# hygenie1228/PoseRisk_RELEASE

Hardware: AMD Instinct MI355X
Metric: frames/sec (224x224 crops) through SPIN ResNet-50 + regressor + SMPL LBS + REBA/RULA (higher is better)
Workload: dtype f32; 1 GPU; configs[1]: batch=64 random 224x224 crops per GPU, ResNet-50+SMPL fp32; global_batch=64, batches_in_flight=3, hipgraph_replay=False, exchange=none, dist_world_size=1

## Files before the change

include/poserisk_hip.h:

```cpp
#ifndef POSERISK_HIP_H
#define POSERISK_HIP_H

#include <stddef.h>
#include <stdint.h>

#ifdef __cplusplus
extern "C" {
#endif

typedef enum pr_status {
  PR_OK = 0,
  PR_ERR_INVALID = -1,
  PR_ERR_HIP = -2,
  PR_ERR_NO_DEVICE = -3,
  PR_ERR_CAPACITY = -4
} pr_status;

const char* pr_last_error(void);
int pr_abi_version(void);
const char* pr_build_info(void);

int pr_declare_stream(void* stream, int declared);

int pr_stem_pool_f32_nhwc(int device, const float* x_dev, const float* w_host, const float* bias_host, float* y_dev, int B,
                          int repeats, float* ms_out, void* stream);

typedef struct pr_hmr pr_hmr_t;

size_t pr_hmr_weight_floats(void);

enum { PR_CONV_FORM_DEFAULT = -1, PR_CONV_FORM_DIRECT = 0, PR_CONV_FORM_WINOGRAD_2X2 = 2, PR_CONV_FORM_WINOGRAD_4X4 = 4,
       PR_CONV_FORM_WINOGRAD_4X4_B = 5, PR_CONV_FORM_BUILTIN_DEFAULT = 5 };
int pr_hmr_create(int device, const float* weights_host, size_t n_floats, int max_batch,
                  int precision, int conv_form, pr_hmr_t** out);
int pr_hmr_destroy(pr_hmr_t* h);

int pr_hmr_forward(pr_hmr_t* h, const float* x_dev, int B, float* rotmat_dev, float* betas_dev,
                   float* cam_dev, float* xf_dev, float* pose6d_dev, void* stream);

int pr_hmr_set_streams(pr_hmr_t* h, int n_streams);

int pr_hmr_set_concurrency(pr_hmr_t* h, int n_in_flight);

int pr_hmr_profile_enable(pr_hmr_t* h, int on);
int pr_hmr_profile_read(pr_hmr_t* h, float* ms_per_layer_host, int* launches_per_layer_host,
                        double* flops_per_layer_per_frame_host, double* mfma_flops_per_layer_per_frame_host,
                        int n_layers);
int pr_hmr_num_conv_layers(void);
int pr_hmr_plan_counts(pr_hmr_t* h, int B, int* conv_launches, int* winograd_layers);
int pr_hmr_encode_until(pr_hmr_t* h, const float* x_dev, int B, int block, void* act_dev, void* stream);
int pr_hmr_regress_until(pr_hmr_t* h, const float* xf_dev, int B, int step, float* out_dev, void* stream);
int pr_hmr_conv_form(pr_hmr_t* h);

int pr_conv_num_tile_cfgs(void);
int pr_conv2d_nhwc(int device, const void* x_dev, const float* w_host, const float* bias_host,
                   const void* res_dev, void* y_dev, int B, int H, int W, int Cin, int Cin_real,
                   int Cout, int KH, int KW, int stride, int pad, int relu, int tile_cfg,
                   int precision, int repeats, float* ms_out, void* stream);

int pr_conv1x1_dual_nhwc(int device, const void* x1_dev, const float* w1_host, const void* x2_dev,
                         const float* w2_host, const float* bias_host, void* y_dev, int B, int Ho, int Wo,
                         int Cin1, int H2, int W2, int Cin2, int stride2, int Cout, int relu, int tile_cfg,
                         int precision, void* stream);

int pr_conv3x3_conv1x1_nhwc(int device, const void* x_dev, const float* w2_host, const float* b2_host,
                            const float* w3_host, const float* b3_host, const void* res_dev, void* y_dev,
                            int B, int H, int W, int Cin, int N3, int relu3, int precision, void* stream);

int pr_bottleneck_nhwc(int device, const void* x_dev, const float* w1_host, const float* b1_host, const float* w2_host,
                       const float* b2_host, const float* w3_host, const float* b3_host, const float* wd_host,
                       const float* bd_host, void* y_dev, int B, int H, int W, int repeats, float* ms_out, void* stream);

int pr_bottleneck128_nhwc(int device, const void* x_dev, const float* w1_host, const float* b1_host, const float* w2_host,
                          const float* b2_host, const float* w3_host, const float* b3_host, void* y_dev, int B, int H, int W,
                          int repeats, float* ms_out, void* stream);

int pr_bottleneck256_nhwc(int device, const void* x_dev, const float* w1_host, const float* b1_host, const float* w2_host,
                          const float* b2_host, const float* w3_host, const float* b3_host, void* y_dev, int B, int H, int W,
                          int repeats, float* ms_out, void* stream);

int pr_stem_pool_nhwc(int device, const void* x_dev, const float* w_host, const float* bias_host, void* y_dev, int B, int H,
                      int repeats, float* ms_out, void* stream);

int pr_crop_frames(const uint8_t* frames_dev, int F, int H, int W, int bgr, const int32_t* frame_idx_dev,
                   const float* bboxes_dev, int N, float scale, float* crops_dev, int32_t* status_dev,
                   void* stream);

int pr_rot6d_to_rotmat(const float* pose6d_dev, int N, float* rotmat_dev, void* stream);

int pr_pose_to_euler(const float* rotmat_dev, int N, float* axis_angle_dev, double* euler_deg_dev,
                     int32_t* status_dev, void* stream);
int pr_axis_angle_to_euler(const float* axis_angle_dev, int N, double* euler_deg_dev, int32_t* status_dev,
                           void* stream);

typedef struct pr_smpl pr_smpl_t;

int pr_smpl_create(int device, const float* v_template_host, const float* shapedirs_host,
                   const float* posedirs_host, const float* J_regressor_host,
                   const float* weights_host, const int32_t* parents_host,
                   const float* model_betas_host, int V, int J, int NB, int max_batch,
                   pr_smpl_t** out);
int pr_smpl_destroy(pr_smpl_t* h);

int pr_smpl_forward(pr_smpl_t* h, const float* pose_dev, const float* betas_dev,
                    const float* trans_dev, int B, int center_idx, float* verts_dev,
                    float* joints_dev, void* stream);

int pr_smpl_joint_cam(pr_smpl_t* h, float* axis_angle_dev, int N, float* joint_cam_dev,
                      float* verts_dev, void* stream);

typedef struct pr_reba_info {
  int32_t legs_bilateral;
  int32_t sitting;
  int32_t load_force;
  int32_t arm_supported_l;
  int32_t arm_supported_r;
  int32_t coupling;
  int32_t activity;
} pr_reba_info;

typedef struct pr_rula_info {
  int32_t arm_supported_l, arm_supported_r;
  int32_t a_muscle_l, a_muscle_r;
  int32_t a_load_l, a_load_r;
  int32_t legs_bilateral;
  int32_t b_muscle, b_load;
} pr_rula_info;

int pr_reba(const double* euler_deg_dev, int N, const pr_reba_info* info, int32_t* out_dev,
            void* stream);
int pr_rula(const double* euler_deg_dev, int N, const pr_rula_info* info, int32_t* out_dev,
            void* stream);

typedef struct pr_frames_out {
  float* rotmat;
  float* betas;
  float* cam;
  float* axis_angle;
  double* euler_deg;
  float* joint_cam;
  float* verts;
  int32_t* reba;
  int32_t* rula;
  int32_t* status;
} pr_frames_out;

int pr_frames_forward(pr_hmr_t* hmr, pr_smpl_t* smpl, const float* x_dev, int B,
                      const pr_reba_info* reba_info, const pr_rula_info* rula_info,
                      const pr_frames_out* out, void* stream);

typedef struct pr_render_args {
  const float* verts;
  const int32_t* faces;
  const float* cam;
  const float* bboxes;
  const uint8_t* frames;
  const int32_t* frame_idx;
  const int32_t* face_part;
  const uint8_t* part_rgb;
  uint8_t* out;
  int32_t* face_id;
  int32_t* vert_fx;
  int32_t* status;
  int N, V, F, P;
  int n_frames, H, W, bgr;
  float scale, alpha;
} pr_render_args;

size_t pr_render_workspace_bytes(int N, int V, int F, int H, int W);
int pr_render_overlay(const pr_render_args* args, void* workspace, size_t workspace_bytes, void* stream);

#ifdef __cplusplus
}
#endif
#endif
```

poserisk_release_amd/_lib.py:

```python
import ctypes as C
import os

HERE = os.path.dirname(os.path.abspath(__file__))
LIB_PATH = os.environ.get("POSERISK_LIB_PATH") or os.path.join(HERE, "libposerisk_hip.so")

ABI_VERSION = 13


class PoseRiskHipError(RuntimeError):
    pass


class RebaInfo(C.Structure):
    _fields_ = [(n, C.c_int32) for n in ("legs_bilateral", "sitting", "load_force", "arm_supported_l",
                                          "arm_supported_r", "coupling", "activity")]


class RulaInfo(C.Structure):
    _fields_ = [(n, C.c_int32) for n in ("arm_supported_l", "arm_supported_r", "a_muscle_l", "a_muscle_r",
                                          "a_load_l", "a_load_r", "legs_bilateral", "b_muscle", "b_load")]


class RenderArgs(C.Structure):
    _fields_ = [(n, C.c_void_p) for n in ("verts", "faces", "cam", "bboxes", "frames", "frame_idx", "face_part", "part_rgb",
                                           "out", "face_id", "vert_fx", "status")] + \
               [(n, C.c_int) for n in ("N", "V", "F", "P", "n_frames", "H", "W", "bgr")] + \
               [("scale", C.c_float), ("alpha", C.c_float)]


class FramesOut(C.Structure):
    _fields_ = [(n, C.c_void_p) for n in ("rotmat", "betas", "cam", "axis_angle", "euler_deg", "joint_cam",
                                           "verts", "reba", "rula", "status")]


_P = C.c_void_p
_I = C.c_int
SIGNATURES = {
    "pr_last_error": (C.c_char_p, []),
    "pr_abi_version": (_I, []),
    "pr_build_info": (C.c_char_p, []),
    "pr_declare_stream": (_I, [_P, _I]),
    "pr_hmr_weight_floats": (C.c_size_t, []),
    "pr_hmr_create": (_I, [_I, _P, C.c_size_t, _I, _I, _I, C.POINTER(_P)]),
    "pr_hmr_destroy": (_I, [_P]),
    "pr_hmr_forward": (_I, [_P, _P, _I, _P, _P, _P, _P, _P, _P]),
    "pr_hmr_set_streams": (_I, [_P, _I]),
    "pr_hmr_set_concurrency": (_I, [_P, _I]),
    "pr_hmr_profile_enable": (_I, [_P, _I]),
    "pr_hmr_profile_read": (_I, [_P, _P, _P, _P, _P, _I]),
    "pr_hmr_num_conv_layers": (_I, []),
    "pr_hmr_conv_form": (_I, [_P]),
    "pr_hmr_plan_counts": (_I, [_P, _I, C.POINTER(_I), C.POINTER(_I)]),
    "pr_hmr_encode_until": (_I, [_P, _P, _I, _I, _P, _P]),
    "pr_hmr_regress_until": (_I, [_P, _P, _I, _I, _P, _P]),
    "pr_conv_num_tile_cfgs": (_I, []),
    "pr_conv2d_nhwc": (_I, [_I, _P, _P, _P, _P, _P] + [_I] * 14 + [_P, _P]),
    "pr_conv1x1_dual_nhwc": (_I, [_I, _P, _P, _P, _P, _P, _P] + [_I] * 12 + [_P]),
    "pr_conv3x3_conv1x1_nhwc": (_I, [_I, _P, _P, _P, _P, _P, _P, _P] + [_I] * 7 + [_P]),
    "pr_bottleneck_nhwc": (_I, [_I, _P, _P, _P, _P, _P, _P, _P, _P, _P, _P, _I, _I, _I, _I, _P, _P]),
    "pr_bottleneck128_nhwc": (_I, [_I, _P, _P, _P, _P, _P, _P, _P, _P, _I, _I, _I, _I, _P, _P]),
    "pr_bottleneck256_nhwc": (_I, [_I, _P, _P, _P, _P, _P, _P, _P, _P, _I, _I, _I, _I, _P, _P]),
    "pr_stem_pool_nhwc": (_I, [_I, _P, _P, _P, _P, _I, _I, _I, _P, _P]),
    "pr_stem_pool_f32_nhwc": (_I, [_I, _P, _P, _P, _P, _I, _I, _P, _P]),
    "pr_crop_frames": (_I, [_P, _I, _I, _I, _I, _P, _P, _I, C.c_float, _P, _P, _P]),
    "pr_rot6d_to_rotmat": (_I, [_P, _I, _P, _P]),
    "pr_pose_to_euler": (_I, [_P, _I, _P, _P, _P, _P]),
    "pr_axis_angle_to_euler": (_I, [_P, _I, _P, _P, _P]),
    "pr_smpl_create": (_I, [_I, _P, _P, _P, _P, _P, _P, _P, _I, _I, _I, _I, C.POINTER(_P)]),
    "pr_smpl_destroy": (_I, [_P]),
    "pr_smpl_forward": (_I, [_P, _P, _P, _P, _I, _I, _P, _P, _P]),
    "pr_smpl_joint_cam": (_I, [_P, _P, _I, _P, _P, _P]),
    "pr_reba": (_I, [_P, _I, C.POINTER(RebaInfo), _P, _P]),
    "pr_rula": (_I, [_P, _I, C.POINTER(RulaInfo), _P, _P]),
    "pr_frames_forward": (_I, [_P, _P, _P, _I, C.POINTER(RebaInfo), C.POINTER(RulaInfo),
                               C.POINTER(FramesOut), _P]),
    "pr_render_workspace_bytes": (C.c_size_t, [_I, _I, _I, _I, _I]),
    "pr_render_overlay": (_I, [C.POINTER(RenderArgs), _P, C.c_size_t, _P]),
}

_lib = None


def load():
    global _lib
    if _lib is not None:
        return _lib
    if not os.path.exists(LIB_PATH):
        raise PoseRiskHipError(
            f"{LIB_PATH} is missing: build it with `python -m poserisk_release_amd.build` "
            "(there is no CPU fallback for the hot path)")
    import torch
    try:
        lib = C.CDLL(LIB_PATH)
    except OSError as e:
        raise PoseRiskHipError(f"cannot load {LIB_PATH}: {e}") from e
    for name, (res, args) in SIGNATURES.items():
        fn = getattr(lib, name)
        fn.restype = res
        fn.argtypes = args
    if lib.pr_abi_version() != ABI_VERSION:
        raise PoseRiskHipError(f"ABI version mismatch: library {lib.pr_abi_version()}, binding {ABI_VERSION}")
    _lib = lib
    return lib


def declare_stream(device=None):
    import torch
    lib = load()
    if torch.cuda.is_available():
        lib.pr_declare_stream(torch.cuda.current_stream(device).cuda_stream, 1)
    return lib


def check(status, what=""):
    if status != 0:
        msg = load().pr_last_error().decode("utf-8", "replace")
        raise PoseRiskHipError(f"{what} failed (status {status}): {msg}")


def reba_info_struct(info):
    return RebaInfo(int(info["Legs_bilateral_weight_bearing/walking"]), int(info["Sitting"]),
                    int(info["Load/Force Score"]), int(info["Arm_supported_leaning_L"]),
                    int(info["Arm_supported_leaning_R"]), int(info["Coupling"]), int(info["Activity_Score"]))


def rula_info_struct(info):
    return RulaInfo(int(info["Arm_supported_leaning_L"]), int(info["Arm_supported_leaning_R"]),
                    int(info["A_Muscle_use_L"]), int(info["A_Muscle_use_R"]), int(info["A_Load/Force_L"]),
                    int(info["A_Load/Force_R"]), int(info["Legs_bilateral_weight_bearing"]),
                    int(info["B_Muscle_use"]), int(info["B_Load/Force"]))
```

poserisk_release_amd/csrc/capi.hip:

```cpp
#include <vector>

#include "conv_igemm.h"
#include "frame_kernels.h"

namespace pr {
namespace {
thread_local std::string g_last_error;
thread_local bool g_stream_declared = false;
thread_local hipStream_t g_declared_stream = nullptr;
}
void declared_stream(bool* declared, hipStream_t* s) {
  *declared = g_stream_declared;
  *s = g_declared_stream;
}
void set_error(const char* fmt, ...) {
  char buf[1024];
  va_list ap;
  va_start(ap, fmt);
  vsnprintf(buf, sizeof buf, fmt, ap);
  va_end(ap);
  g_last_error = buf;
}
}

#define PR_STR_(x) #x
#define PR_STR(x) PR_STR_(x)

extern "C" {

const char* pr_last_error(void) { return pr::g_last_error.c_str(); }
int pr_abi_version(void) { return 13; }

int pr_declare_stream(void* stream, int declared) {
  pr::g_stream_declared = declared != 0;
  pr::g_declared_stream = declared ? (hipStream_t)stream : nullptr;
  return PR_OK;
}

const char* pr_build_info(void) {
  return "gfx950"
#ifdef PR_TIMING_HOOKS
         " +PR_TIMING_HOOKS(results may be wrong)"
#endif
#ifdef PR_EXPERIMENT
         " +PR_EXPERIMENT=" PR_STR(PR_EXPERIMENT)
#endif
#if !defined(PR_TIMING_HOOKS) && !defined(PR_EXPERIMENT)
         " release"
#endif
      ;
}

int pr_rot6d_to_rotmat(const float* pose6d_dev, int N, float* rotmat_dev, void* stream) {
  PR_REQUIRE(pose6d_dev && rotmat_dev && N >= 0, "pr_rot6d_to_rotmat: bad argument");
  return pr::launch_rot6d(pose6d_dev, rotmat_dev, (long)N * 24, (hipStream_t)stream);
}

int pr_pose_to_euler(const float* rotmat_dev, int N, float* axis_angle_dev, double* euler_deg_dev,
                     int32_t* status_dev, void* stream) {
  PR_REQUIRE(rotmat_dev && axis_angle_dev && euler_deg_dev && N >= 0, "pr_pose_to_euler: bad argument");
  return pr::launch_pose_to_euler(rotmat_dev, N, axis_angle_dev, euler_deg_dev, status_dev,
                                  (hipStream_t)stream);
}

int pr_axis_angle_to_euler(const float* axis_angle_dev, int N, double* euler_deg_dev, int32_t* status_dev,
                           void* stream) {
  PR_REQUIRE(axis_angle_dev && euler_deg_dev && N >= 0, "pr_axis_angle_to_euler: bad argument");
  return pr::launch_pose_to_euler(nullptr, N, const_cast<float*>(axis_angle_dev), euler_deg_dev, status_dev,
                                  (hipStream_t)stream);
}

int pr_reba(const double* euler_deg_dev, int N, const pr_reba_info* info, int32_t* out_dev, void* stream) {
  PR_REQUIRE(euler_deg_dev && info && out_dev && N >= 0, "pr_reba: bad argument");
  return pr::launch_reba(euler_deg_dev, N, *info, out_dev, (hipStream_t)stream);
}

int pr_rula(const double* euler_deg_dev, int N, const pr_rula_info* info, int32_t* out_dev, void* stream) {
  PR_REQUIRE(euler_deg_dev && info && out_dev && N >= 0, "pr_rula: bad argument");
  return pr::launch_rula(euler_deg_dev, N, *info, out_dev, (hipStream_t)stream);
}

int pr_crop_frames(const uint8_t* frames_dev, int F, int H, int W, int bgr, const int32_t* frame_idx_dev,
                   const float* bboxes_dev, int N, float scale, float* crops_dev, int32_t* status_dev,
                   void* stream) {
  PR_REQUIRE(frames_dev && bboxes_dev && crops_dev, "pr_crop_frames: null argument");
  PR_REQUIRE(F > 0 && H > 0 && W > 0 && H < 32768 && W < 32768 && N >= 0 && scale > 0, "pr_crop_frames: bad geometry");
  PR_REQUIRE(frame_idx_dev || N <= F, "pr_crop_frames: %d boxes for %d frames without a frame index", N, F);
  return pr::launch_crop_frames(frames_dev, F, H, W, bgr, frame_idx_dev, bboxes_dev, N, scale, crops_dev,
                                status_dev, (hipStream_t)stream);
}

int pr_conv_num_tile_cfgs(void) { return pr::conv_num_tile_cfgs(); }

int pr_conv2d_nhwc(int device, const void* x_dev, const float* w_host, const float* bias_host,
                   const void* res_dev, void* y_dev, int B, int H, int W, int Cin, int Cin_real, int Cout,
                   int KH, int KW, int stride, int pad, int relu, int tile_cfg, int precision, int repeats,
                   float* ms_out, void* stream) {
  using namespace pr;
  PR_REQUIRE(x_dev && w_host && y_dev, "pr_conv2d_nhwc: null argument");
  PR_REQUIRE(precision == 0 || precision == 1, "pr_conv2d_nhwc: precision %d unknown", precision);
  PR_REQUIRE(precision == 0 || Cin % 8 == 0, "pr_conv2d_nhwc: bf16 needs Cin %% 8 == 0");
  PR_REQUIRE(Cin_real > 0 && Cin_real <= Cin && Cout % 64 == 0, "pr_conv2d_nhwc: bad channels");
  PR_REQUIRE(stride > 0 && pad >= 0 && KH > 0 && KW > 0, "pr_conv2d_nhwc: bad geometry");
  DeviceGuard g(device);
  hipStream_t s = (hipStream_t)stream;
  PR_TRY(refuse_if_capturing(s, "stand-alone test entry"));
  ConvProblem p;
  p.B = B; p.H = H; p.W = W; p.Cin = Cin; p.Cout = Cout; p.KH = KH; p.KW = KW; p.stride = stride; p.pad = pad;
  p.Ho = (H + 2 * pad - KH) / stride + 1;
  p.Wo = (W + 2 * pad - KW) / stride + 1;
  p.relu = relu;
  PR_REQUIRE(p.Ho > 0 && p.Wo > 0, "pr_conv2d_nhwc: empty output");
  p.precision = precision;
  p.tune = conv_tuning_from_env();
  struct Scratch {
    float *wd = nullptr, *bd = nullptr, *work = nullptr, *slab = nullptr;
    int* tickets = nullptr;
    hipEvent_t e0 = nullptr, e1 = nullptr;
    ~Scratch() {
      if (slab) (void)hipFree(slab);
      if (tickets) (void)hipFree(tickets);
      if (wd) (void)hipFree(wd);
      if (bd) (void)hipFree(bd);
      if (work) (void)hipFree(work);
      if (e0) (void)hipEventDestroy(e0);
      if (e1) (void)hipEventDestroy(e1);
    }
  } sc;
  float *&wd = sc.wd, *&bd = sc.bd, *&work = sc.work;
  const bool wino = tile_cfg == -2 || tile_cfg == -4 || tile_cfg == -5;
  const int wino_m = -tile_cfg;
  if (wino) {
    PR_REQUIRE(precision == 0 && KH == 3 && KW == 3 && stride == 1 && pad == 1 && !res_dev && Cin == Cin_real &&
                   Cin % 32 == 0,
               "pr_conv2d_nhwc: tile_cfg -2 / -4 / -5 (Winograd) is for fp32 3x3 / stride 1 / pad 1 without residual, Cin %% 32 == 0");
    const int wn = conv_winograd_tile(wino_m) + 2;
    std::vector<float> u((size_t)wn * wn * Cout * Cin);
    conv_winograd_pack_weights(w_host, nullptr, Cout, Cin, wino_m, u.data());
    PR_HIP(hipMalloc(&wd, u.size() * sizeof(float)));
    PR_HIP(hipMemcpy(wd, u.data(), u.size() * sizeof(float), hipMemcpyHostToDevice));
    PR_HIP(hipMalloc(&work, std::max<size_t>(conv_winograd_work_floats(p, wino_m), 4) * sizeof(float)));
  } else if (precision == 1) {
    std::vector<unsigned short> packed((size_t)Cout * conv_kpad_bf16(p.K()));
    conv_pack_weights_bf16(w_host, nullptr, Cout, Cin_real, Cin, KH, KW, packed.data());
    PR_HIP(hipMalloc(&wd, packed.size() * 2));
    PR_HIP(hipMemcpy(wd, packed.data(), packed.size() * 2, hipMemcpyHostToDevice));
  } else {
    std::vector<float> packed((size_t)Cout * p.Kpad());
    conv_pack_weights(w_host, nullptr, Cout, Cin_real, Cin, KH, KW, packed.data());
    PR_HIP(hipMalloc(&wd, packed.size() * sizeof(float)));
    PR_HIP(hipMemcpy(wd, packed.data(), packed.size() * sizeof(float), hipMemcpyHostToDevice));
  }
  if (bias_host) {
    PR_HIP(hipMalloc(&bd, Cout * sizeof(float)));
    PR_HIP(hipMemcpy(bd, bias_host, Cout * sizeof(float), hipMemcpyHostToDevice));
  }
  p.x = (const float*)x_dev; p.w = wd; p.bias = bd; p.res = (const float*)res_dev; p.y = (float*)y_dev;
  int cfg = tile_cfg >= 0 ? tile_cfg : conv_pick_tile_cfg(p);
  if (tile_cfg > 200 && tile_cfg <= 208) {
    PR_REQUIRE(precision == 0, "pr_conv2d_nhwc: split-K is fp32 only");
    cfg = 8;
    p.splitk = tile_cfg - 200;
    const size_t tiles = (size_t)ceil_div(p.M(), 64) * (Cout / 64);
    PR_HIP(hipMalloc(&sc.slab, tiles * p.splitk * 4096 * sizeof(float)));
    PR_HIP(hipMalloc(&sc.tickets, tiles * sizeof(int)));
    p.split_slab = sc.slab;
    p.split_tickets = sc.tickets;
  }
  auto go = [&]() -> int { return wino ? conv_winograd_launch(p, wd, work, wino_m, s) : conv_launch(p, cfg, s); };
  int st = go();
  if (st == PR_OK && repeats > 0 && ms_out) {
    hipEvent_t &e0 = sc.e0, &e1 = sc.e1;
    PR_HIP(hipEventCreate(&e0));
    PR_HIP(hipEventCreate(&e1));
    PR_HIP(hipEventRecord(e0, s));
    for (int i = 0; i < repeats && st == PR_OK; ++i) st = go();
    PR_HIP(hipEventRecord(e1, s));
    PR_HIP(hipEventSynchronize(e1));
    float ms = 0.f;
    PR_HIP(hipEventElapsedTime(&ms, e0, e1));
    *ms_out = ms / repeats;
  }
  hipError_t e = hipStreamSynchronize(s);
  if (st != PR_OK) return st;
  PR_HIP(e);
  return PR_OK;
}

int pr_conv1x1_dual_nhwc(int device, const void* x1_dev, const float* w1_host, const void* x2_dev, const float* w2_host,
                         const float* bias_host, void* y_dev, int B, int Ho, int Wo, int Cin1, int H2, int W2, int Cin2,
                         int stride2, int Cout, int relu, int tile_cfg, int precision, void* stream) {
  using namespace pr;
  PR_REQUIRE(x1_dev && w1_host && x2_dev && w2_host && y_dev, "pr_conv1x1_dual_nhwc: null argument");
  PR_REQUIRE(precision == 0 || precision == 1, "pr_conv1x1_dual_nhwc: precision %d unknown", precision);
  const int kq = precision == 1 ? 64 : kConvBK;
  PR_REQUIRE(Cin1 > 0 && Cin2 > 0 && Cin1 % kq == 0 && Cin2 % kq == 0 && Cout % 64 == 0 && stride2 > 0,
             "pr_conv1x1_dual_nhwc: channels must be multiples of %d (Cout of 64)", kq);
  DeviceGuard g(device);
  hipStream_t s = (hipStream_t)stream;
  PR_TRY(refuse_if_capturing(s, "stand-alone test entry"));
  ConvProblem p;
  p.B = B; p.H = p.Ho = Ho; p.W = p.Wo = Wo; p.Cin = Cin1; p.Cout = Cout; p.KH = p.KW = 1; p.stride = 1; p.pad = 0;
  p.relu = relu; p.precision = precision;
  p.tune = conv_tuning_from_env();
  p.H2 = H2; p.W2 = W2; p.Cin2 = Cin2; p.stride2 = stride2;
  struct Scratch {
    float *wd = nullptr, *bd = nullptr;
    ~Scratch() {
      if (wd) (void)hipFree(wd);
      if (bd) (void)hipFree(bd);
    }
  } sc;
  const size_t K = (size_t)Cin1 + Cin2;
  if (precision == 1) {
    std::vector<unsigned short> a((size_t)Cout * Cin1), b((size_t)Cout * Cin2), packed((size_t)Cout * K);
    conv_pack_weights_bf16(w1_host, nullptr, Cout, Cin1, Cin1, 1, 1, a.data());
    conv_pack_weights_bf16(w2_host, nullptr, Cout, Cin2, Cin2, 1, 1, b.data());
    for (int o = 0; o < Cout; ++o) {
      memcpy(&packed[o * K], &a[(size_t)o * Cin1], (size_t)Cin1 * 2);
      memcpy(&packed[o * K + Cin1], &b[(size_t)o * Cin2], (size_t)Cin2 * 2);
    }
    PR_HIP(hipMalloc(&sc.wd, packed.size() * 2));
    PR_HIP(hipMemcpy(sc.wd, packed.data(), packed.size() * 2, hipMemcpyHostToDevice));
  } else {
    std::vector<float> packed((size_t)Cout * K);
    for (int o = 0; o < Cout; ++o) {
      memcpy(&packed[o * K], w1_host + (size_t)o * Cin1, (size_t)Cin1 * 4);
      memcpy(&packed[o * K + Cin1], w2_host + (size_t)o * Cin2, (size_t)Cin2 * 4);
    }
    PR_HIP(hipMalloc(&sc.wd, packed.size() * 4));
    PR_HIP(hipMemcpy(sc.wd, packed.data(), packed.size() * 4, hipMemcpyHostToDevice));
  }
  if (bias_host) {
    PR_HIP(hipMalloc(&sc.bd, Cout * sizeof(float)));
    PR_HIP(hipMemcpy(sc.bd, bias_host, Cout * sizeof(float), hipMemcpyHostToDevice));
  }
  p.x = (const float*)x1_dev; p.x2 = (const float*)x2_dev; p.w = sc.wd; p.bias = sc.bd; p.res = nullptr; p.y = (float*)y_dev;
  const int cfg = tile_cfg >= 0 ? tile_cfg : conv_pick_tile_cfg(p);
  const int st = conv_launch(p, cfg, s);
  const hipError_t e = hipStreamSynchronize(s);
  if (st != PR_OK) return st;
  PR_HIP(e);
  return PR_OK;
}

int pr_conv3x3_conv1x1_nhwc(int device, const void* x_dev, const float* w2_host, const float* b2_host,
                            const float* w3_host, const float* b3_host, const void* res_dev, void* y_dev, int B, int H,
                            int W, int Cin, int N3, int relu3, int precision, void* stream) {
  using namespace pr;
  PR_REQUIRE(x_dev && w2_host && b2_host && w3_host && b3_host && y_dev, "pr_conv3x3_conv1x1_nhwc: null argument");
  PR_REQUIRE(precision == 0 || precision == 1, "pr_conv3x3_conv1x1_nhwc: precision %d unknown", precision);
  PR_REQUIRE(Cin >= (precision ? 64 : 32) && (Cin & (Cin - 1)) == 0 && N3 > 0 && N3 % 64 == 0,
             "pr_conv3x3_conv1x1_nhwc: Cin must be a power of two >= 32 (bf16: 64), N3 a multiple of 64");
  DeviceGuard g(device);
  hipStream_t s = (hipStream_t)stream;
  PR_TRY(refuse_if_capturing(s, "stand-alone test entry"));
  struct Scratch {
    float* p[4] = {nullptr, nullptr, nullptr, nullptr};
    ~Scratch() {
      for (float* q : p)
        if (q) (void)hipFree(q);
    }
  } sc;
  ConvProblem p;
  p.B = B; p.H = p.Ho = H; p.W = p.Wo = W; p.Cin = Cin; p.Cout = 64; p.KH = p.KW = 3; p.stride = 1; p.pad = 1; p.relu = 1;
  p.precision = precision;
  p.tune = conv_tuning_from_env();
  std::vector<float> w2p, w3p;
  if (precision == 1) {
    std::vector<unsigned short> a((size_t)64 * conv_kpad_bf16(p.K())), b((size_t)N3 * 64);
    conv_pack_weights_bf16(w2_host, nullptr, 64, Cin, Cin, 3, 3, a.data());
    conv_pack_weights_bf16(w3_host, nullptr, N3, 64, 64, 1, 1, b.data());
    w2p.resize((a.size() + 1) / 2);
    w3p.resize((b.size() + 1) / 2);
    memcpy(w2p.data(), a.data(), a.size() * 2);
    memcpy(w3p.data(), b.data(), b.size() * 2);
  } else {
    w2p.resize((size_t)64 * p.Kpad());
    conv_pack_weights(w2_host, nullptr, 64, Cin, Cin, 3, 3, w2p.data());
    w3p.assign(w3_host, w3_host + (size_t)N3 * 64);
  }
  const size_t sizes[4] = {w2p.size(), 64, w3p.size(), (size_t)N3};
  const float* src[4] = {w2p.data(), b2_host, w3p.data(), b3_host};
  for (int i = 0; i < 4; ++i) {
    PR_HIP(hipMalloc(&sc.p[i], sizes[i] * sizeof(float)));
    PR_HIP(hipMemcpy(sc.p[i], src[i], sizes[i] * sizeof(float), hipMemcpyHostToDevice));
  }
  p.x = (const float*)x_dev; p.w = sc.p[0]; p.bias = sc.p[1]; p.w3 = sc.p[2]; p.bias3 = sc.p[3];
  p.res3 = (const float*)res_dev; p.y3 = (float*)y_dev;
  p.N3 = N3; p.relu3 = relu3;
  const int st = conv_launch(p, 8, s);
  const hipError_t e = hipStreamSynchronize(s);
  if (st != PR_OK) return st;
  PR_HIP(e);
  return PR_OK;
}

int pr_bottleneck_nhwc(int device, const void* x_dev, const float* w1_host, const float* b1_host, const float* w2_host,
                       const float* b2_host, const float* w3_host, const float* b3_host, const float* wd_host,
                       const float* bd_host, void* y_dev, int B, int H, int W, int repeats, float* ms_out, void* stream) {
  using namespace pr;
  PR_REQUIRE(x_dev && w1_host && b1_host && w2_host && b2_host && w3_host && b3_host && y_dev, "pr_bottleneck_nhwc: null argument");
  PR_REQUIRE(!wd_host == !bd_host, "pr_bottleneck_nhwc: the downsample branch needs both its weight and its bias");
  PR_REQUIRE(B >= 0 && H > 0 && W > 0, "pr_bottleneck_nhwc: bad geometry");
  const bool first = wd_host != nullptr;
  const int cin = first ? 64 : 256, k3 = first ? 128 : 64;
  DeviceGuard g(device);
  hipStream_t s = (hipStream_t)stream;
  PR_TRY(refuse_if_capturing(s, "stand-alone test entry"));
  struct Scratch {
    void* p[6] = {};
    hipEvent_t e0 = nullptr, e1 = nullptr;
    ~Scratch() {
      for (void* q : p)
        if (q) (void)hipFree(q);
      if (e0) (void)hipEventDestroy(e0);
      if (e1) (void)hipEventDestroy(e1);
    }
  } sc;
  std::vector<unsigned short> a1((size_t)64 * cin), a2((size_t)64 * 576), a3((size_t)256 * 64), ad((size_t)256 * 64),
      a3d((size_t)256 * k3), p1(a1.size()), p2(a2.size()), p3(a3d.size());
  conv_pack_weights_bf16(w1_host, nullptr, 64, cin, cin, 1, 1, a1.data());
  conv_pack_weights_bf16(w2_host, nullptr, 64, 64, 64, 3, 3, a2.data());
  conv_pack_weights_bf16(w3_host, nullptr, 256, 64, 64, 1, 1, a3.data());
  if (first) conv_pack_weights_bf16(wd_host, nullptr, 256, 64, 64, 1, 1, ad.data());
  for (int o = 0; o < 256; ++o) {
    memcpy(&a3d[(size_t)o * k3], &a3[(size_t)o * 64], 128);
    if (first) memcpy(&a3d[(size_t)o * k3 + 64], &ad[(size_t)o * 64], 128);
  }
  std::vector<float> b3(b3_host, b3_host + 256);
  if (first)
    for (int o = 0; o < 256; ++o) b3[o] = (float)((double)b3_host[o] + (double)bd_host[o]);
  bottleneck_pack_rows_bf16(a1.data(), 64, cin, p1.data());
  bottleneck_pack_rows_bf16(a2.data(), 64, 576, p2.data());
  bottleneck_pack_rows_bf16(a3d.data(), 256, k3, p3.data());
  const void* src[6] = {p1.data(), p2.data(), p3.data(), b1_host, b2_host, b3.data()};
  const size_t bytes[6] = {p1.size() * 2, p2.size() * 2, p3.size() * 2, 64 * 4, 64 * 4, 256 * 4};
  for (int i = 0; i < 6; ++i) {
    PR_HIP(hipMalloc(&sc.p[i], bytes[i]));
    PR_HIP(hipMemcpy(sc.p[i], src[i], bytes[i], hipMemcpyHostToDevice));
  }
  BottleneckProblem p;
  p.x = x_dev; p.y = y_dev; p.w1 = sc.p[0]; p.w2 = sc.p[1]; p.w3 = sc.p[2];
  p.b1 = (const float*)sc.p[3]; p.b2 = (const float*)sc.p[4]; p.b3 = (const float*)sc.p[5];
  p.B = B; p.H = H; p.W = W; p.first = first;
  int st = bottleneck_bf16_launch(p, s);
  if (st == PR_OK && repeats > 0 && ms_out) {
    PR_HIP(hipEventCreate(&sc.e0));
    PR_HIP(hipEventCreate(&sc.e1));
    PR_HIP(hipEventRecord(sc.e0, s));
    for (int i = 0; i < repeats && st == PR_OK; ++i) st = bottleneck_bf16_launch(p, s);
    PR_HIP(hipEventRecord(sc.e1, s));
    PR_HIP(hipEventSynchronize(sc.e1));
    float ms = 0.f;
    PR_HIP(hipEventElapsedTime(&ms, sc.e0, sc.e1));
    *ms_out = ms / repeats;
  }
  const hipError_t e = hipStreamSynchronize(s);
  if (st != PR_OK) return st;
  PR_HIP(e);
  return PR_OK;
}

int pr_bottleneck128_nhwc(int device, const void* x_dev, const float* w1_host, const float* b1_host, const float* w2_host,
                          const float* b2_host, const float* w3_host, const float* b3_host, void* y_dev, int B, int H, int W,
                          int repeats, float* ms_out, void* stream) {
  using namespace pr;
  PR_REQUIRE(x_dev && w1_host && b1_host && w2_host && b2_host && w3_host && b3_host && y_dev, "pr_bottleneck128_nhwc: null argument");
  PR_REQUIRE(B >= 0 && H > 0 && W > 0, "pr_bottleneck128_nhwc: bad geometry");
  DeviceGuard g(device);
  hipStream_t s = (hipStream_t)stream;
  PR_TRY(refuse_if_capturing(s, "stand-alone test entry"));
  struct Scratch {
    void* p[6] = {};
    hipEvent_t e0 = nullptr, e1 = nullptr;
    ~Scratch() {
      for (void* q : p)
        if (q) (void)hipFree(q);
      if (e0) (void)hipEventDestroy(e0);
      if (e1) (void)hipEventDestroy(e1);
    }
  } sc;
  std::vector<unsigned short> a1((size_t)128 * 512), a2((size_t)128 * 1152), a3((size_t)512 * 128), p1(a1.size()), p2(a2.size()),
      p3(a3.size());
  conv_pack_weights_bf16(w1_host, nullptr, 128, 512, 512, 1, 1, a1.data());
  conv_pack_weights_bf16(w2_host, nullptr, 128, 128, 128, 3, 3, a2.data());
  conv_pack_weights_bf16(w3_host, nullptr, 512, 128, 128, 1, 1, a3.data());
  bottleneck_pack_rows_bf16(a1.data(), 128, 512, p1.data());
  bottleneck_pack_rows_bf16(a2.data(), 128, 1152, p2.data());
  bottleneck_pack_rows_bf16(a3.data(), 512, 128, p3.data());
  const void* src[6] = {p1.data(), p2.data(), p3.data(), b1_host, b2_host, b3_host};
  const size_t bytes[6] = {p1.size() * 2, p2.size() * 2, p3.size() * 2, 128 * 4, 128 * 4, 512 * 4};
  for (int i = 0; i < 6; ++i) {
    PR_HIP(hipMalloc(&sc.p[i], bytes[i]));
    PR_HIP(hipMemcpy(sc.p[i], src[i], bytes[i], hipMemcpyHostToDevice));
  }
  BottleneckProblem p;
  p.x = x_dev; p.y = y_dev; p.w1 = sc.p[0]; p.w2 = sc.p[1]; p.w3 = sc.p[2];
  p.b1 = (const float*)sc.p[3]; p.b2 = (const float*)sc.p[4]; p.b3 = (const float*)sc.p[5];
  p.B = B; p.H = H; p.W = W; p.planes = 128; p.first = false;
  int st = bottleneck_bf16_launch(p, s);
  if (st == PR_OK && repeats > 0 && ms_out) {
    PR_HIP(hipEventCreate(&sc.e0));
    PR_HIP(hipEventCreate(&sc.e1));
    PR_HIP(hipEventRecord(sc.e0, s));
    for (int i = 0; i < repeats && st == PR_OK; ++i) st = bottleneck_bf16_launch(p, s);
    PR_HIP(hipEventRecord(sc.e1, s));
    PR_HIP(hipEventSynchronize(sc.e1));
    float ms = 0.f;
    PR_HIP(hipEventElapsedTime(&ms, sc.e0, sc.e1));
    *ms_out = ms / repeats;
  }
  const hipError_t e = hipStreamSynchronize(s);
  if (st != PR_OK) return st;
  PR_HIP(e);
  return PR_OK;
}

int pr_bottleneck256_nhwc(int device, const void* x_dev, const float* w1_host, const float* b1_host, const float* w2_host,
                          const float* b2_host, const float* w3_host, const float* b3_host, void* y_dev, int B, int H, int W,
                          int repeats, float* ms_out, void* stream) {
  using namespace pr;
  PR_REQUIRE(x_dev && w1_host && b1_host && w2_host && b2_host && w3_host && b3_host && y_dev, "pr_bottleneck256_nhwc: null argument");
  PR_REQUIRE(B >= 0 && H > 0 && W > 0, "pr_bottleneck256_nhwc: bad geometry");
  DeviceGuard g(device);
  hipStream_t s = (hipStream_t)stream;
  PR_TRY(refuse_if_capturing(s, "stand-alone test entry"));
  struct Scratch {
    void* p[6] = {};
    hipEvent_t e0 = nullptr, e1 = nullptr;
    ~Scratch() {
      for (void* q : p)
        if (q) (void)hipFree(q);
      if (e0) (void)hipEventDestroy(e0);
      if (e1) (void)hipEventDestroy(e1);
    }
  } sc;
  std::vector<unsigned short> a1((size_t)256 * 1024), a2((size_t)256 * 2304), a3((size_t)1024 * 256), p1(a1.size()), p2(a2.size()),
      p3(a3.size()), rows(a2.size());
  conv_pack_weights_bf16(w1_host, nullptr, 256, 1024, 1024, 1, 1, a1.data());
  conv_pack_weights_bf16(w2_host, nullptr, 256, 256, 256, 3, 3, a2.data());
  conv_pack_weights_bf16(w3_host, nullptr, 1024, 256, 256, 1, 1, a3.data());
  bottleneck_pack_rows_bf16(a1.data(), 256, 1024, p1.data());
  bottleneck_pack_rows_bf16(a2.data(), 256, 2304, rows.data());
  bottleneck256_pack_w2_frags_bf16(rows.data(), p2.data());
  bottleneck_pack_rows_bf16(a3.data(), 1024, 256, rows.data());
  bottleneck256_pack_w3_frags_bf16(rows.data(), p3.data());
  const void* src[6] = {p1.data(), p2.data(), p3.data(), b1_host, b2_host, b3_host};
  const size_t bytes[6] = {p1.size() * 2, p2.size() * 2, p3.size() * 2, 256 * 4, 256 * 4, 1024 * 4};
  for (int i = 0; i < 6; ++i) {
    PR_HIP(hipMalloc(&sc.p[i], bytes[i]));
    PR_HIP(hipMemcpy(sc.p[i], src[i], bytes[i], hipMemcpyHostToDevice));
  }
  BottleneckProblem p;
  p.x = x_dev; p.y = y_dev; p.w1 = sc.p[0]; p.w2 = sc.p[1]; p.w3 = sc.p[2];
  p.b1 = (const float*)sc.p[3]; p.b2 = (const float*)sc.p[4]; p.b3 = (const float*)sc.p[5];
  p.B = B; p.H = H; p.W = W; p.planes = 256; p.first = false;
  int st = bottleneck_bf16_launch(p, s);
  if (st == PR_OK && repeats > 0 && ms_out) {
    PR_HIP(hipEventCreate(&sc.e0));
    PR_HIP(hipEventCreate(&sc.e1));
    PR_HIP(hipEventRecord(sc.e0, s));
    for (int i = 0; i < repeats && st == PR_OK; ++i) st = bottleneck_bf16_launch(p, s);
    PR_HIP(hipEventRecord(sc.e1, s));
    PR_HIP(hipEventSynchronize(sc.e1));
    float ms = 0.f;
    PR_HIP(hipEventElapsedTime(&ms, sc.e0, sc.e1));
    *ms_out = ms / repeats;
  }
  const hipError_t e = hipStreamSynchronize(s);
  if (st != PR_OK) return st;
  PR_HIP(e);
  return PR_OK;
}

int pr_stem_pool_nhwc(int device, const void* x_dev, const float* w_host, const float* bias_host, void* y_dev, int B, int H,
                      int repeats, float* ms_out, void* stream) {
  using namespace pr;
  PR_REQUIRE(x_dev && w_host && bias_host && y_dev, "pr_stem_pool_nhwc: null argument");
  DeviceGuard g(device);
  hipStream_t s = (hipStream_t)stream;
  PR_TRY(refuse_if_capturing(s, "stand-alone test entry"));
  struct Scratch {
    void* p[2] = {};
    hipEvent_t e0 = nullptr, e1 = nullptr;
    ~Scratch() {
      for (void* q : p)
        if (q) (void)hipFree(q);
      if (e0) (void)hipEventDestroy(e0);
      if (e1) (void)hipEventDestroy(e1);
    }
  } sc;
  std::vector<unsigned short> packed((size_t)64 * 256);
  conv_pack_weights_bf16(w_host, nullptr, 64, 16, 16, 4, 4, packed.data());
  PR_HIP(hipMalloc(&sc.p[0], packed.size() * 2));
  PR_HIP(hipMemcpy(sc.p[0], packed.data(), packed.size() * 2, hipMemcpyHostToDevice));
  PR_HIP(hipMalloc(&sc.p[1], 64 * 4));
  PR_HIP(hipMemcpy(sc.p[1], bias_host, 64 * 4, hipMemcpyHostToDevice));
  int st = stem_pool_bf16_launch(x_dev, sc.p[0], (const float*)sc.p[1], y_dev, B, H, s);
  if (st == PR_OK && repeats > 0 && ms_out) {
    PR_HIP(hipEventCreate(&sc.e0));
    PR_HIP(hipEventCreate(&sc.e1));
    PR_HIP(hipEventRecord(sc.e0, s));
    for (int i = 0; i < repeats && st == PR_OK; ++i) st = stem_pool_bf16_launch(x_dev, sc.p[0], (const float*)sc.p[1], y_dev, B, H, s);
    PR_HIP(hipEventRecord(sc.e1, s));
    PR_HIP(hipEventSynchronize(sc.e1));
    float ms = 0.f;
    PR_HIP(hipEventElapsedTime(&ms, sc.e0, sc.e1));
    *ms_out = ms / repeats;
  }
  const hipError_t e = hipStreamSynchronize(s);
  if (st != PR_OK) return st;
  PR_HIP(e);
  return PR_OK;
}

int pr_stem_pool_f32_nhwc(int device, const float* x_dev, const float* w_host, const float* bias_host, float* y_dev, int B,
                          int repeats, float* ms_out, void* stream) {
  using namespace pr;
  PR_REQUIRE(x_dev && w_host && bias_host && y_dev, "pr_stem_pool_f32_nhwc: null argument");
  DeviceGuard g(device);
  hipStream_t s = (hipStream_t)stream;
  PR_TRY(refuse_if_capturing(s, "stand-alone test entry"));
  struct Scratch {
    void* p[2] = {};
    hipEvent_t e0 = nullptr, e1 = nullptr;
    ~Scratch() {
      for (void* q : p)
        if (q) (void)hipFree(q);
      if (e0) (void)hipEventDestroy(e0);
      if (e1) (void)hipEventDestroy(e1);
    }
  } sc;
  for (int o = 0; o < 64; ++o)
    for (int c12 = 0; c12 < 12; ++c12)
      for (int t = 0; t < 4; ++t) {
        const int sub = c12 / 3;
        const float top = w_host[((o * 12 + c12) * 4 + 0) * 4 + t], left = w_host[((o * 12 + c12) * 4 + t) * 4 + 0];
        PR_REQUIRE(((sub >> 1) != 0 || top == 0.f) && ((sub & 1) != 0 || left == 0.f),
                   "pr_stem_pool_f32_nhwc: the weights must be a 7x7 kernel in the 4x4 taps' 8x8 window (zero for tap row 0 / "
                   "sub-row 0 and for tap column 0 / sub-column 0); output channel %d, channel %d is not", o, c12);
      }
  std::vector<float> packed((size_t)64 * 192);
  conv_pack_weights(w_host, nullptr, 64, 12, 12, 4, 4, packed.data());
  PR_HIP(hipMalloc(&sc.p[0], packed.size() * 4));
  PR_HIP(hipMemcpy(sc.p[0], packed.data(), packed.size() * 4, hipMemcpyHostToDevice));
  PR_HIP(hipMalloc(&sc.p[1], 64 * 4));
  PR_HIP(hipMemcpy(sc.p[1], bias_host, 64 * 4, hipMemcpyHostToDevice));
  int st = stem_pool_f32_launch(x_dev, (const float*)sc.p[0], (const float*)sc.p[1], y_dev, B, s);
  if (st == PR_OK && repeats > 0 && ms_out) {
    PR_HIP(hipEventCreate(&sc.e0));
    PR_HIP(hipEventCreate(&sc.e1));
    PR_HIP(hipEventRecord(sc.e0, s));
    for (int i = 0; i < repeats && st == PR_OK; ++i) st = stem_pool_f32_launch(x_dev, (const float*)sc.p[0], (const float*)sc.p[1], y_dev, B, s);
    PR_HIP(hipEventRecord(sc.e1, s));
    PR_HIP(hipEventSynchronize(sc.e1));
    float ms = 0.f;
    PR_HIP(hipEventElapsedTime(&ms, sc.e0, sc.e1));
    *ms_out = ms / repeats;
  }
  const hipError_t e = hipStreamSynchronize(s);
  if (st != PR_OK) return st;
  PR_HIP(e);
  return PR_OK;
}

int pr_frames_forward(pr_hmr_t* hmr, pr_smpl_t* smpl, const float* x_dev, int B,
                      const pr_reba_info* reba_info, const pr_rula_info* rula_info,
                      const pr_frames_out* out, void* stream) {
  PR_REQUIRE(B >= 0, "pr_frames_forward: negative batch");
  if (B == 0) return PR_OK;
  PR_REQUIRE(hmr && smpl && x_dev && out, "pr_frames_forward: null argument");
  PR_REQUIRE(out->rotmat && out->axis_angle && out->euler_deg && out->joint_cam,
             "pr_frames_forward: rotmat, axis_angle, euler_deg and joint_cam are required");
  PR_REQUIRE((!out->reba || reba_info) && (!out->rula || rula_info), "pr_frames_forward: score output without info");
  PR_TRY(pr_hmr_forward(hmr, x_dev, B, out->rotmat, out->betas, out->cam, nullptr, nullptr, stream));
  PR_TRY(pr_pose_to_euler(out->rotmat, B, out->axis_angle, out->euler_deg, out->status, stream));
  PR_TRY(pr_smpl_joint_cam(smpl, out->axis_angle, B, out->joint_cam, out->verts, stream));
  if (out->reba) PR_TRY(pr_reba(out->euler_deg, B, reba_info, out->reba, stream));
  if (out->rula) PR_TRY(pr_rula(out->euler_deg, B, rula_info, out->rula, stream));
  return PR_OK;
}

}
```

poserisk_release_amd/csrc/conv_igemm.h:

```cpp
#pragma once
#include "common.h"
#include "host_plan.h"

namespace pr {


struct ConvTuning {
  int force_cfg = -1;
  int tail = 1;
  int tail_min_rounds = 2;
  int tail_max_rem = 128;
  int wino_vec = 2;
  int wino_bm = 64, wino_bn = 64;
  int wino_regw = 1;
  int regw_per_cu = 2;
  int regw_wt = 0, regw_wnb = 0;
  int regw_t = 0, regw_nb = 0;
  int bal_stages = 4;
};
ConvTuning conv_tuning_from_env();

struct ConvProblem {
  const float* x;
  const float* w;
  const float* bias;
  const float* res;
  float* y;
  int B, H, W, Cin, Ho, Wo, Cout, KH, KW, stride, pad;
  int relu;
  int precision = 0;
  int groups = 1;
  const float* x2 = nullptr;
  int H2 = 0, W2 = 0, Cin2 = 0, stride2 = 1;
  const float* w3 = nullptr;
  const float* bias3 = nullptr;
  const float* res3 = nullptr;
  float* y3 = nullptr;
  int N3 = 0, relu3 = 0;
  int splitk = 1;
  float* split_slab = nullptr;
  int* split_tickets = nullptr;
  ConvTuning tune;
  int M() const { return B * Ho * Wo; }
  int K() const { return KH * KW * Cin; }
  int Kpad() const { return ceil_div(K(), kConvBK) * kConvBK; }
  double flops() const { return 2.0 * (double)M() * (Cout * (K() + (x2 ? Cin2 : 0)) + (w3 ? (double)N3 * Cout : 0.0)); }
};

int conv_num_tile_cfgs();
const char* conv_tile_cfg_name(int cfg);
int conv_pick_tile_cfg(const ConvProblem& p);
int conv_launch(const ConvProblem& p, int cfg, hipStream_t stream);

int conv_fused3_launch(const ConvProblem& p, hipStream_t stream);

int conv_panel_launch(const ConvProblem& p, hipStream_t stream);

int conv_dma_launch(const ConvProblem& p, int BM, int BN, hipStream_t stream, int threads = 0);

int conv_dma_bf16_launch(const ConvProblem& p, int BM, int BN, hipStream_t stream, int threads = 0);
int conv_tile_dims(int cfg, int* BM, int* BN);

size_t conv_winograd_work_floats(const ConvProblem& p, int form);
int conv_winograd_launch(const ConvProblem& p, const float* u, float* work, int form, hipStream_t stream);

struct BottleneckProblem {
  const void* x = nullptr;
  void* y = nullptr;
  const void *w1 = nullptr, *w2 = nullptr, *w3 = nullptr;
  const float *b1 = nullptr, *b2 = nullptr, *b3 = nullptr;
  int B = 0, H = 0, W = 0, planes = 64;
  bool first = false;
  int lead_tiles = 2;
  double flops() const { return 2.0 * B * H * W * (double)planes * planes * (first ? 1 + 9 + 8 : 4 + 9 + 4); }
};
int bottleneck_bf16_launch(const BottleneckProblem& p, hipStream_t stream);
int bottleneck128_bf16_launch(const BottleneckProblem& p, hipStream_t stream);
int bottleneck256_bf16_launch(const BottleneckProblem& p, hipStream_t stream);

int stem_pool_bf16_launch(const void* x_s2d, const void* w, const float* bias, void* y, int B, int H, hipStream_t stream);

int stem_pool_f32_launch(const float* x_s2d, const float* w, const float* bias, float* y, int B, hipStream_t stream);

int expand_dual_bf16_launch(const void* t, const void* x2, const void* w, const float* bias, void* y, int B, int Ho, int Wo, int H2,
                            int W2, int stride2, int K1, int K2, int N, int relu, hipStream_t stream);
int expand_res_bf16_launch(const void* t, const void* w, const float* bias, const void* res, void* y, long M, int K, int N,
                           int relu, hipStream_t stream);

bool conv_bal_bf16_fits(const ConvProblem& p);
bool conv_bal_bf16_pays(const ConvProblem& p, int cus);
int conv_bal_bf16_launch(const ConvProblem& p, hipStream_t stream, int variant = 0);

bool conv_regw_f32_fits(const ConvProblem& p);
int conv_regw_f32_launch(const ConvProblem& p, hipStream_t stream);

}
```

poserisk_release_amd/csrc/conv_winograd.hip:

```cpp
#include <algorithm>

#include "conv_igemm.h"

namespace pr {
namespace {

using f32x4 = __attribute__((ext_vector_type(4))) float;

struct WinoArgs {
  const float* x;
  float* v;
  const float* m;
  const float* bias;
  float* y;
  int B, H, W, C, Cout, th, tw, relu;
  long P;
};

__global__ __launch_bounds__(256) void wino_input_transform(const WinoArgs a) {
  const int c4n = a.C >> 2;
  const long idx = xcd_contiguous_block(blockIdx.x, gridDim.x) * 256 + threadIdx.x;
  if (idx >= a.P * c4n) return;
  const long p = idx / c4n;
  const int c = (int)(idx - p * c4n) * 4;
  const int tx = (int)(p % a.tw);
  const long q = p / a.tw;
  const int ty = (int)(q % a.th), img = (int)(q / a.th);
  const int h0 = 2 * ty - 1, w0 = 2 * tx - 1;
  f32x4 d[4][4];
#pragma unroll
  for (int i = 0; i < 4; ++i)
#pragma unroll
    for (int j = 0; j < 4; ++j) {
      const int hi = h0 + i, wi = w0 + j;
      const bool ok = (unsigned)hi < (unsigned)a.H && (unsigned)wi < (unsigned)a.W;
      const f32x4 z = {0.f, 0.f, 0.f, 0.f};
      d[i][j] = ok ? *reinterpret_cast<const f32x4*>(a.x + (((long)img * a.H + hi) * a.W + wi) * a.C + c) : z;
    }
  f32x4 t[4][4];
#pragma unroll
  for (int j = 0; j < 4; ++j) {
    t[0][j] = d[0][j] - d[2][j];
    t[1][j] = d[1][j] + d[2][j];
    t[2][j] = d[2][j] - d[1][j];
    t[3][j] = d[1][j] - d[3][j];
  }
  const long gs = a.P * a.C;
  float* out = a.v + p * a.C + c;
#pragma unroll
  for (int i = 0; i < 4; ++i) {
    *reinterpret_cast<f32x4*>(out + (4 * i + 0) * gs) = t[i][0] - t[i][2];
    *reinterpret_cast<f32x4*>(out + (4 * i + 1) * gs) = t[i][1] + t[i][2];
    *reinterpret_cast<f32x4*>(out + (4 * i + 2) * gs) = t[i][2] - t[i][1];
    *reinterpret_cast<f32x4*>(out + (4 * i + 3) * gs) = t[i][1] - t[i][3];
  }
}

__global__ __launch_bounds__(256) void wino_output_transform(const WinoArgs a) {
  const int c4n = a.Cout >> 2;
  const long idx = xcd_contiguous_block(blockIdx.x, gridDim.x) * 256 + threadIdx.x;
  if (idx >= a.P * c4n) return;
  const long p = idx / c4n;
  const int c = (int)(idx - p * c4n) * 4;
  const int tx = (int)(p % a.tw);
  const long q = p / a.tw;
  const int ty = (int)(q % a.th), img = (int)(q / a.th);
  const long gs = a.P * a.Cout;
  const float* in = a.m + p * a.Cout + c;
  f32x4 m[4][4];
#pragma unroll
  for (int i = 0; i < 4; ++i)
#pragma unroll
    for (int j = 0; j < 4; ++j) m[i][j] = *reinterpret_cast<const f32x4*>(in + (4 * i + j) * gs);
  f32x4 s[2][4];
#pragma unroll
  for (int j = 0; j < 4; ++j) {
    s[0][j] = (m[0][j] + m[1][j]) + m[2][j];
    s[1][j] = (m[1][j] - m[2][j]) - m[3][j];
  }
  f32x4 b = {0.f, 0.f, 0.f, 0.f};
  if (a.bias) b = *reinterpret_cast<const f32x4*>(a.bias + c);
#pragma unroll
  for (int i = 0; i < 2; ++i) {
    const int ho = 2 * ty + i;
    if (ho >= a.H) continue;
    f32x4 o[2];
    o[0] = ((s[i][0] + s[i][1]) + s[i][2]) + b;
    o[1] = ((s[i][1] - s[i][2]) - s[i][3]) + b;
#pragma unroll
    for (int j = 0; j < 2; ++j) {
      const int wo = 2 * tx + j;
      if (wo >= a.W) continue;
      f32x4 v = o[j];
      if (a.relu) {
        v[0] = fmaxf(v[0], 0.f); v[1] = fmaxf(v[1], 0.f); v[2] = fmaxf(v[2], 0.f); v[3] = fmaxf(v[3], 0.f);
      }
      *reinterpret_cast<f32x4*>(a.y + (((long)img * a.H + ho) * a.W + wo) * a.Cout + c) = v;
    }
  }
}


using f32x2 = __attribute__((ext_vector_type(2))) float;

constexpr float kWa2 = kWa * kWa, kWb2 = kWb * kWb, kWab2 = kWa2 * kWb2, kWs2 = kWa2 + kWb2;

template <int PTS, typename V>
__device__ __forceinline__ void bt6(V& a0, V& a1, V& a2, V& a3, V& a4, V& a5) {
  const V d0 = a0, d1 = a1, d2 = a2, d3 = a3, d4 = a4, d5 = a5;
  if constexpr (PTS == 0) {
    a0 = 4.f * d0 - 5.f * d2 + d4;
    a1 = (d3 + d4) - 4.f * (d1 + d2);
    a2 = 4.f * (d1 - d2) + (d4 - d3);
    a3 = 2.f * (d3 - d1) + (d4 - d2);
    a4 = 2.f * (d1 - d3) + (d4 - d2);
    a5 = 4.f * d1 - 5.f * d3 + d5;
  } else {
    const V ea = d4 - kWb2 * d2, oa = kWa * (d3 - kWb2 * d1);
    const V eb = d4 - kWa2 * d2, ob = kWb * (d3 - kWa2 * d1);
    a0 = (kWab2 * d0 - kWs2 * d2) + d4;
    a1 = ea + oa;
    a2 = ea - oa;
    a3 = eb + ob;
    a4 = eb - ob;
    a5 = (kWab2 * d1 - kWs2 * d3) + d5;
  }
}

template <int PTS, typename V>
__global__ __launch_bounds__(256) void wino43_input_transform(const WinoArgs a) {
  constexpr int NC = sizeof(V) / 4;
  const int c2n = a.C / NC;
  const long idx = xcd_contiguous_block(blockIdx.x, gridDim.x) * 256 + threadIdx.x;
  if (idx >= a.P * c2n) return;
  const long p = idx / c2n;
  const int c = (int)(idx - p * c2n) * NC;
  const int tx = (int)(p % a.tw);
  const long q = p / a.tw;
  const int ty = (int)(q % a.th), img = (int)(q / a.th);
  const int h0 = 4 * ty - 1, w0 = 4 * tx - 1;
  V d[6][6];
#pragma unroll
  for (int i = 0; i < 6; ++i)
#pragma unroll
    for (int j = 0; j < 6; ++j) {
      const int hi = h0 + i, wi = w0 + j;
      const bool ok = (unsigned)hi < (unsigned)a.H && (unsigned)wi < (unsigned)a.W;
      V z;
#pragma unroll
      for (int e = 0; e < NC; ++e) z[e] = 0.f;
      d[i][j] = ok ? *reinterpret_cast<const V*>(a.x + (((long)img * a.H + hi) * a.W + wi) * a.C + c) : z;
    }
#pragma unroll
  for (int j = 0; j < 6; ++j) bt6<PTS>(d[0][j], d[1][j], d[2][j], d[3][j], d[4][j], d[5][j]);
#pragma unroll
  for (int i = 0; i < 6; ++i) bt6<PTS>(d[i][0], d[i][1], d[i][2], d[i][3], d[i][4], d[i][5]);
  const long gs = a.P * a.C;
  float* out = a.v + p * a.C + c;
#pragma unroll
  for (int i = 0; i < 6; ++i)
#pragma unroll
    for (int j = 0; j < 6; ++j) *reinterpret_cast<V*>(out + (6 * i + j) * gs) = d[i][j];
}

template <int PTS, typename V>
__device__ __forceinline__ void at6(const V m0, const V m1, const V m2, const V m3, const V m4, const V m5, V& o0, V& o1, V& o2, V& o3) {
  const V s12 = m1 + m2, d12 = m1 - m2, s34 = m3 + m4, d34 = m3 - m4;
  o0 = (m0 + s12) + s34;
  if constexpr (PTS == 0) {
    o1 = d12 + 2.f * d34;
    o2 = s12 + 4.f * s34;
    o3 = (d12 + 8.f * d34) + m5;
  } else {
    o1 = kWa * d12 + kWb * d34;
    o2 = kWa2 * s12 + kWb2 * s34;
    o3 = ((kWa2 * kWa) * d12 + (kWb2 * kWb) * d34) + m5;
  }
}

template <int PTS, typename V>
__global__ __launch_bounds__(256) void wino43_output_transform(const WinoArgs a) {
  constexpr int NC = sizeof(V) / 4;
  const int c2n = a.Cout / NC;
  const long idx = xcd_contiguous_block(blockIdx.x, gridDim.x) * 256 + threadIdx.x;
  if (idx >= a.P * c2n) return;
  const long p = idx / c2n;
  const int c = (int)(idx - p * c2n) * NC;
  const int tx = (int)(p % a.tw);
  const long q = p / a.tw;
  const int ty = (int)(q % a.th), img = (int)(q / a.th);
  const long gs = a.P * a.Cout;
  const float* in = a.m + p * a.Cout + c;
  V s[4][6];
#pragma unroll
  for (int j = 0; j < 6; ++j) {
    V m[6];
#pragma unroll
    for (int i = 0; i < 6; ++i) m[i] = *reinterpret_cast<const V*>(in + (6 * i + j) * gs);
    at6<PTS>(m[0], m[1], m[2], m[3], m[4], m[5], s[0][j], s[1][j], s[2][j], s[3][j]);
  }
  V b;
#pragma unroll
  for (int e = 0; e < NC; ++e) b[e] = 0.f;
  if (a.bias) b = *reinterpret_cast<const V*>(a.bias + c);
#pragma unroll
  for (int i = 0; i < 4; ++i) {
    const int ho = 4 * ty + i;
    V o[4];
    at6<PTS>(s[i][0], s[i][1], s[i][2], s[i][3], s[i][4], s[i][5], o[0], o[1], o[2], o[3]);
    if (ho >= a.H) continue;
#pragma unroll
    for (int j = 0; j < 4; ++j) {
      const int wo = 4 * tx + j;
      if (wo >= a.W) continue;
      V v = o[j] + b;
      if (a.relu) {
#pragma unroll
        for (int e = 0; e < NC; ++e) v[e] = fmaxf(v[e], 0.f);
      }
      *reinterpret_cast<V*>(a.y + (((long)img * a.H + ho) * a.W + wo) * a.Cout + c) = v;
    }
  }
}

long wino_tiles(const ConvProblem& p, int m) { return (long)p.B * ((p.H + m - 1) / m) * ((p.W + m - 1) / m); }

}

size_t conv_winograd_work_floats(const ConvProblem& p, int form) {
  const int m = conv_winograd_tile(form);
  return (size_t)(m + 2) * (m + 2) * wino_tiles(p, m) * ((size_t)p.Cin + p.Cout);
}

int conv_winograd_launch(const ConvProblem& p, const float* u, float* work, int form, hipStream_t stream) {
  PR_REQUIRE(form == 2 || form == 4 || form == 5, "winograd: form %d (2 = F(2x2), 4 = F(4x4), 5 = F(4x4) on the points 0, +-11/16, +-3/2)", form);
  const int m_out = conv_winograd_tile(form);
  PR_REQUIRE(p.precision == 0 && p.KH == 3 && p.KW == 3 && p.stride == 1 && p.pad == 1 && !p.res,
             "winograd: 3x3 / stride 1 / pad 1 fp32 convolutions without residual only");
  PR_REQUIRE(p.Cin % kConvBK == 0 && p.Cout % 64 == 0, "winograd: Cin %% 32 and Cout %% 64 (got %d, %d)", p.Cin, p.Cout);
  PR_REQUIRE(p.x && p.y && u && work, "winograd: null tensor");
  if (p.B == 0) return PR_OK;
  const int n2 = (m_out + 2) * (m_out + 2);
  WinoArgs a;
  a.x = p.x; a.bias = p.bias; a.y = p.y;
  a.B = p.B; a.H = p.H; a.W = p.W; a.C = p.Cin; a.Cout = p.Cout; a.relu = p.relu;
  a.th = (p.H + m_out - 1) / m_out; a.tw = (p.W + m_out - 1) / m_out;
  a.P = wino_tiles(p, m_out);
  a.v = work;
  float* m = work + (size_t)n2 * a.P * p.Cin;
  a.m = m;
  PR_REQUIRE(a.P * std::max(p.Cin, p.Cout) < (1L << 29), "winograd: %ld tiles are too many for one launch", a.P);
  const bool wide = m_out == 4 && p.tune.wino_vec == 4;
  const int per = m_out == 4 ? (wide ? 4 : 2) : 4;
  const long n_in = a.P * (p.Cin / per), n_out = a.P * (p.Cout / per);
  if (form == 5 && wide) hipLaunchKernelGGL((wino43_input_transform<1, f32x4>), dim3((unsigned)ceil_div(n_in, 256L)), dim3(256), 0, stream, a);
  else if (form == 5) hipLaunchKernelGGL((wino43_input_transform<1, f32x2>), dim3((unsigned)ceil_div(n_in, 256L)), dim3(256), 0, stream, a);
  else if (m_out == 4 && wide) hipLaunchKernelGGL((wino43_input_transform<0, f32x4>), dim3((unsigned)ceil_div(n_in, 256L)), dim3(256), 0, stream, a);
  else if (m_out == 4) hipLaunchKernelGGL((wino43_input_transform<0, f32x2>), dim3((unsigned)ceil_div(n_in, 256L)), dim3(256), 0, stream, a);
  else hipLaunchKernelGGL(wino_input_transform, dim3((unsigned)ceil_div(n_in, 256L)), dim3(256), 0, stream, a);
  PR_TRY(check_launch("wino_input_transform"));
  ConvProblem g;
  g.x = work; g.w = u; g.bias = nullptr; g.res = nullptr; g.y = m;
  g.B = (int)a.P; g.H = g.W = g.Ho = g.Wo = 1; g.Cin = p.Cin; g.Cout = p.Cout;
  g.KH = g.KW = 1; g.stride = 1; g.pad = 0; g.relu = 0; g.precision = 0;
  g.groups = n2;
  g.tune = p.tune;
  PR_REQUIRE(p.Cout % p.tune.wino_bn == 0, "winograd: Cout %d is not a multiple of the grouped GEMM's tile N %d", p.Cout, p.tune.wino_bn);
  if (p.tune.wino_regw && conv_regw_f32_fits(g)) PR_TRY(conv_regw_f32_launch(g, stream));
  else PR_TRY(conv_dma_launch(g, p.tune.wino_bm, p.tune.wino_bn, stream, 256));
  if (form == 5 && wide) hipLaunchKernelGGL((wino43_output_transform<1, f32x4>), dim3((unsigned)ceil_div(n_out, 256L)), dim3(256), 0, stream, a);
  else if (form == 5) hipLaunchKernelGGL((wino43_output_transform<1, f32x2>), dim3((unsigned)ceil_div(n_out, 256L)), dim3(256), 0, stream, a);
  else if (m_out == 4 && wide) hipLaunchKernelGGL((wino43_output_transform<0, f32x4>), dim3((unsigned)ceil_div(n_out, 256L)), dim3(256), 0, stream, a);
  else if (m_out == 4) hipLaunchKernelGGL((wino43_output_transform<0, f32x2>), dim3((unsigned)ceil_div(n_out, 256L)), dim3(256), 0, stream, a);
  else hipLaunchKernelGGL(wino_output_transform, dim3((unsigned)ceil_div(n_out, 256L)), dim3(256), 0, stream, a);
  return check_launch("wino_output_transform");
}

}
```

poserisk_release_amd/csrc/hmr.hip:

```cpp
#include <algorithm>
#include <cmath>
#include <cstdlib>
#include <cstring>
#include <memory>
#include <vector>

#include "conv_igemm.h"
#include "frame_kernels.h"

struct pr_hmr : pr::HmrPlan {
  int device = 0;
  pr::ConvTuning tune;
  float* split_slab[8] = {};
  int* split_tickets[8] = {};
  std::vector<float*> dev_allocs;
  static constexpr int kMaxChunks = pr::kHmrMaxChunks;
  int n_chunks = 1;
  int chunk_cap = 0;
  float* act[kMaxChunks][6] = {};
  float* wino_work[kMaxChunks] = {};
  hipStream_t streams[kMaxChunks] = {};
  hipEvent_t ev_fork = nullptr;
  hipEvent_t ev_join[kMaxChunks] = {};
  std::vector<float*> act_allocs;
  bool profile = false;
  std::vector<float> prof_ms;
  std::vector<int> prof_n;
  std::vector<std::pair<hipEvent_t, hipEvent_t>> pending;
  std::vector<int> pending_layer;
};

namespace pr {
namespace {

struct DeviceSink : PlanSink {
  pr_hmr* h;
  explicit DeviceSink(pr_hmr* handle) : h(handle) {}
  int upload(const void* host, size_t bytes, float** out) override {
    float* d = nullptr;
    PR_HIP(hipMalloc(&d, std::max<size_t>(bytes, 16)));
    h->dev_allocs.push_back(d);
    PR_HIP(hipMemcpy(d, host, bytes, hipMemcpyHostToDevice));
    *out = d;
    return PR_OK;
  }
  int zeros(size_t bytes, float** out) override {
    float* d = nullptr;
    PR_HIP(hipMalloc(&d, std::max<size_t>(bytes, 16)));
    h->dev_allocs.push_back(d);
    PR_HIP(hipMemset(d, 0, std::max<size_t>(bytes, 16)));
    *out = d;
    return PR_OK;
  }
};

int set_chunks(pr_hmr* h, int n) {
  PR_REQUIRE(n >= 1 && n <= pr_hmr::kMaxChunks, "hmr: stream count %d out of range 1..%d", n, pr_hmr::kMaxChunks);
  PR_HIP(hipDeviceSynchronize());
  for (float* p : h->act_allocs) (void)hipFree(p);
  h->act_allocs.clear();
  h->n_chunks = n;
  h->chunk_cap = hmr_chunk_cap(h->max_batch, n);
  const HmrChunkSizes z = hmr_chunk_sizes(*h, h->chunk_cap);
  for (int c = 0; c < n; ++c) {
    for (int i = 0; i <= 5; ++i) {
      float* d = nullptr;
      PR_HIP(hipMalloc(&d, (i == 0 ? z.act0_floats : z.act_floats) * sizeof(float)));
      h->act_allocs.push_back(d);
      h->act[c][i] = d;
    }
    if (z.wino_floats) {
      float* d = nullptr;
      PR_HIP(hipMalloc(&d, z.wino_floats * sizeof(float)));
      h->act_allocs.push_back(d);
      h->wino_work[c] = d;
    }
    if (z.slab_floats) {
      float* d = nullptr;
      PR_HIP(hipMalloc(&d, z.slab_floats * sizeof(float)));
      h->act_allocs.push_back(d);
      h->split_slab[c] = d;
      PR_HIP(hipMalloc(&d, z.tickets * sizeof(int)));
      h->act_allocs.push_back(d);
      h->split_tickets[c] = reinterpret_cast<int*>(d);
    }
    if (n > 1 && !h->streams[c]) PR_HIP(hipStreamCreateWithFlags(&h->streams[c], hipStreamNonBlocking));
    if (n > 1 && !h->ev_join[c]) PR_HIP(hipEventCreateWithFlags(&h->ev_join[c], hipEventDisableTiming));
  }
  if (n > 1 && !h->ev_fork) PR_HIP(hipEventCreateWithFlags(&h->ev_fork, hipEventDisableTiming));
  return PR_OK;
}

ConvProblem conv_problem(const pr_hmr* h, const ConvSpec& c, int chunk, int B) {
  ConvProblem p;
  p.x = h->act[chunk][c.in_buf];
  p.w = c.w;
  p.bias = c.bias;
  p.res = c.res_buf >= 0 ? h->act[chunk][c.res_buf] : nullptr;
  p.y = h->act[chunk][c.out_buf];
  p.B = B; p.H = c.H; p.W = c.W; p.Cin = c.Cin; p.Ho = c.Ho(); p.Wo = c.Wo(); p.Cout = c.Cout;
  p.KH = p.KW = c.k; p.stride = c.stride; p.pad = c.pad; p.relu = c.relu;
  p.precision = h->precision;
  p.tune = h->tune;
  if (c.in2_buf >= 0) {
    p.x2 = h->act[chunk][c.in2_buf];
    p.H2 = p.W2 = c.H2; p.Cin2 = c.Cin2; p.stride2 = c.stride2;
  }
  if (c.splitk > 1) {
    p.splitk = c.splitk;
    p.split_slab = h->split_slab[chunk];
    p.split_tickets = h->split_tickets[chunk];
  }
  if (c.w3 && c.out3_buf >= 0) {
    p.w3 = c.w3; p.bias3 = c.bias3; p.N3 = c.N3; p.relu3 = 1;
    p.res3 = c.res3_buf >= 0 ? h->act[chunk][c.res3_buf] : nullptr;
    p.y3 = h->act[chunk][c.out3_buf];
  }
  return p;
}

int fc_launch(const pr_hmr* h, const FcSpec& fc, const float* x, const float* res, float* y, int B, bool use_bias,
              hipStream_t s) {
  if (!h->fc_tiles) return launch_fc_rows16(x, fc.w, use_bias ? fc.bias : nullptr, res, y, B, fc.N, fc.K, s, h->fc_shape);
  ConvProblem p;
  p.x = x; p.w = fc.w; p.bias = use_bias ? fc.bias : nullptr; p.res = res; p.y = y;
  p.B = B; p.H = p.W = p.Ho = p.Wo = 1; p.Cin = fc.K; p.Cout = fc.N;
  p.KH = p.KW = 1; p.stride = 1; p.pad = 0; p.relu = 0;
  p.tune = h->tune;
  return conv_launch(p, conv_pick_tile_cfg(p), s);
}


struct ChunkRun {
  int chunk;
  const float* x;
  int b;
  float* xf_out;
  hipStream_t s;
  void* tap = nullptr;
};

size_t block_frame_elems(int k) {
  if (k == 0) return (size_t)56 * 56 * 64;
  const int L = k <= 3 ? 0 : k <= 7 ? 1 : k <= 13 ? 2 : 3, hw = 56 >> L;
  return (size_t)hw * hw * (256 << L);
}

int encode_chunks(pr_hmr* h, const ChunkRun* runs, int n, int stop_block = -1) {
  const bool bf = h->precision == 1;
  for (int i = 0; i < n; ++i) {
    if (h->stem_s2d) {
      if (bf) PR_TRY(launch_nchw3_to_s2d16_bf16(runs[i].x, h->act[runs[i].chunk][0], runs[i].b, kImg, kImg, runs[i].s));
      else PR_TRY(launch_nchw3_to_s2d12(runs[i].x, h->act[runs[i].chunk][0], runs[i].b, kImg, kImg, runs[i].s));
    } else {
      if (bf) PR_TRY(launch_nchw3_to_nhwc8_bf16(runs[i].x, h->act[runs[i].chunk][0], runs[i].b, kImg, kImg, runs[i].s));
      else PR_TRY(launch_nchw3_to_nhwc4(runs[i].x, h->act[runs[i].chunk][0], runs[i].b, kImg, kImg, runs[i].s));
    }
  }
  auto fused_pays = [&](int b) { return hmr_fused3_pays(b, h->cus); };
  size_t skip_until[pr_hmr::kMaxChunks] = {};
  for (size_t ci = 0; ci < h->convs.size(); ++ci) {
    ConvSpec& c = h->convs[ci];
    const int li = c.layer;
    const pr::HmrPlan::FusedBlock* alt = nullptr;
    for (const pr::HmrPlan::FusedBlock& fb : h->fused3)
      if (fb.first == ci) alt = &fb;
    for (int i = 0; i < n; ++i) {
      const ChunkRun& r = runs[i];
      if (ci < skip_until[i]) continue;
      if (alt && fused_pays(r.b)) {
        BottleneckProblem bp;
        bp.x = h->act[r.chunk][alt->blk.in_buf]; bp.y = h->act[r.chunk][alt->blk.out_buf];
        bp.w1 = alt->blk.w; bp.w2 = alt->blk.w2b; bp.w3 = alt->blk.w3;
        bp.b1 = alt->blk.bias; bp.b2 = alt->blk.bias2b; bp.b3 = alt->blk.bias3;
        bp.B = r.b; bp.H = alt->blk.H; bp.W = alt->blk.W; bp.planes = alt->blk.bneck_planes; bp.first = false;
        if (h->profile) {
          hipEvent_t e0, e1;
          PR_HIP(hipEventCreate(&e0));
          PR_HIP(hipEventCreate(&e1));
          PR_HIP(hipEventRecord(e0, r.s));
          PR_TRY(bottleneck_bf16_launch(bp, r.s));
          PR_HIP(hipEventRecord(e1, r.s));
          h->pending.emplace_back(e0, e1);
          h->pending_layer.push_back(alt->blk.layer);
        } else {
          PR_TRY(bottleneck_bf16_launch(bp, r.s));
        }
        skip_until[i] = ci + 3;
        continue;
      }
      ConvProblem p = c.bneck_planes ? ConvProblem{} : conv_problem(h, c, r.chunk, r.b);
      int cfg = c.cfg >= 0 || c.bneck_planes ? c.cfg : conv_pick_tile_cfg(p);
      if (bf && h->balanced && c.cfg < 0 && !c.bneck_planes && !c.u && conv_bal_bf16_pays(p, h->cus)) cfg = kConvCfgBalanced;
      const bool stem_pool = ci == 0 && h->stem_s2d && h->fuse_stem;
      auto go = [&]() -> int {
        if (stem_pool && !bf)
          return stem_pool_f32_launch(h->act[r.chunk][0], c.w, c.bias, h->act[r.chunk][2], r.b, r.s);
        if (stem_pool)
          return stem_pool_bf16_launch(h->act[r.chunk][0], c.w, c.bias, h->act[r.chunk][2], r.b, kImg / 2, r.s);
        if (c.bneck_planes) {
          BottleneckProblem bp;
          bp.x = h->act[r.chunk][c.in_buf]; bp.y = h->act[r.chunk][c.out_buf];
          bp.w1 = c.w; bp.w2 = c.w2b; bp.w3 = c.w3; bp.b1 = c.bias; bp.b2 = c.bias2b; bp.b3 = c.bias3;
          bp.B = r.b; bp.H = c.H; bp.W = c.W; bp.planes = c.bneck_planes; bp.first = c.bneck_first;
          bp.lead_tiles = h->b128_lead;
          return bottleneck_bf16_launch(bp, r.s);
        }
        return c.u ? conv_winograd_launch(p, c.u, h->wino_work[r.chunk], c.wino_form, r.s) : conv_launch(p, cfg, r.s);
      };
      if (h->profile) {
        hipEvent_t e0, e1;
        PR_HIP(hipEventCreate(&e0));
        PR_HIP(hipEventCreate(&e1));
        PR_HIP(hipEventRecord(e0, r.s));
        PR_TRY(go());
        PR_HIP(hipEventRecord(e1, r.s));
        h->pending.emplace_back(e0, e1);
        h->pending_layer.push_back(li);
      } else {
        PR_TRY(go());
      }
      if (ci == 0 && !stem_pool) {
        if (bf) PR_TRY(launch_maxpool_bf16(h->act[r.chunk][1], h->act[r.chunk][2], r.b, 112, 112, 64, r.s));
        else PR_TRY(launch_maxpool(h->act[r.chunk][1], h->act[r.chunk][2], r.b, 112, 112, 64, r.s));
      }
    }
    if (stop_block >= 0 && ci == (size_t)h->block_last[stop_block]) {
      const size_t frame_bytes = block_frame_elems(stop_block) * (bf ? 2 : 4);
      for (int i = 0; i < n; ++i)
        PR_HIP(hipMemcpyAsync(runs[i].tap, h->act[runs[i].chunk][h->block_buf[stop_block]], runs[i].b * frame_bytes,
                              hipMemcpyDeviceToDevice, runs[i].s));
      return PR_OK;
    }
  }
  for (int i = 0; i < n; ++i) {
    if (bf) PR_TRY(launch_avgpool_bf16(h->act[runs[i].chunk][h->final_buf], runs[i].xf_out, runs[i].b, 49, 2048, runs[i].s));
    else PR_TRY(launch_avgpool(h->act[runs[i].chunk][h->final_buf], runs[i].xf_out, runs[i].b, 49, 2048, runs[i].s));
  }
  return PR_OK;
}

}
}

extern "C" {

size_t pr_hmr_weight_floats(void) { return pr::hmr_weight_floats(); }
int pr_hmr_num_conv_layers(void) { return pr::kNumConv; }

int pr_hmr_create(int device, const float* weights_host, size_t n_floats, int max_batch, int precision,
                  int conv_form, pr_hmr_t** out) {
  using namespace pr;
  PR_REQUIRE(out && weights_host, "pr_hmr_create: null argument");
  PR_REQUIRE(max_batch > 0 && max_batch <= 4096, "pr_hmr_create: max_batch %d out of range", max_batch);
  PR_REQUIRE(precision == 0 || precision == 1, "pr_hmr_create: precision %d unknown (0 = fp32, 1 = bf16 encoder)", precision);
  PR_REQUIRE(hmr_conv_form_valid(conv_form),
             "pr_hmr_create: conv_form %d unknown (-1 default, 0 direct, 2 F(2x2,3x3), 4 F(4x4,3x3), 5 F(4x4,3x3) on the "
             "points 0, +-11/16, +-3/2, or three digits of those for layer2 / layer3 / layer4)", conv_form);
  PR_REQUIRE(n_floats == hmr_weight_floats(), "pr_hmr_create: blob has %zu floats, expected %zu", n_floats,
             hmr_weight_floats());
  int ndev = 0;
  if (hipGetDeviceCount(&ndev) != hipSuccess || ndev <= 0) {
    set_error("pr_hmr_create: no HIP device visible");
    return PR_ERR_NO_DEVICE;
  }
  PR_REQUIRE(device >= 0 && device < ndev, "pr_hmr_create: device %d of %d", device, ndev);
  DeviceGuard g(device);
  PR_TRY(refuse_under_declared_capture("pr_hmr_create"));
  std::unique_ptr<pr_hmr> h(new pr_hmr);
  h->device = device;
  hmr_plan_configure(h.get(), precision, conv_form, max_batch);
  h->tune = conv_tuning_from_env();
  (void)hipDeviceGetAttribute(&h->cus, hipDeviceAttributeMultiprocessorCount, h->device);
  DeviceSink sink(h.get());
  int st = hmr_plan_build(h.get(), weights_host, n_floats, sink);
  h->prof_ms.assign(kNumConv, 0.f);
  h->prof_n.assign(kNumConv, 0);
  if (st == PR_OK) {
    int n = 1;
    if (const char* e = getenv("POSERISK_HMR_STREAMS")) n = atoi(e);
    n = std::max(1, std::min(n, (int)pr_hmr::kMaxChunks));
    st = set_chunks(h.get(), std::min(n, max_batch));
  }
  if (st != PR_OK) {
    for (float* p : h->dev_allocs) (void)hipFree(p);
    for (float* p : h->act_allocs) (void)hipFree(p);
    return st;
  }
  *out = h.release();
  return PR_OK;
}

int pr_hmr_destroy(pr_hmr_t* h) {
  if (!h) return PR_OK;
  pr::DeviceGuard g(h->device);
  PR_TRY(pr::refuse_under_declared_capture("pr_hmr_destroy"));
  for (auto& pe : h->pending) {
    (void)hipEventDestroy(pe.first);
    (void)hipEventDestroy(pe.second);
  }
  for (float* p : h->dev_allocs) (void)hipFree(p);
  for (float* p : h->act_allocs) (void)hipFree(p);
  for (int c = 0; c < pr_hmr::kMaxChunks; ++c) {
    if (h->streams[c]) (void)hipStreamDestroy(h->streams[c]);
    if (h->ev_join[c]) (void)hipEventDestroy(h->ev_join[c]);
  }
  if (h->ev_fork) (void)hipEventDestroy(h->ev_fork);
  delete h;
  return PR_OK;
}

int pr_hmr_set_concurrency(pr_hmr_t* h, int n_in_flight) {
  PR_REQUIRE(h, "pr_hmr_set_concurrency: null handle");
  PR_REQUIRE(n_in_flight >= 1, "pr_hmr_set_concurrency: %d handles in flight", n_in_flight);
  if (!getenv("POSERISK_REGW_PER_CU")) h->tune.regw_per_cu = n_in_flight >= 2 ? 1 : 2;
  return PR_OK;
}

int pr_hmr_set_streams(pr_hmr_t* h, int n_streams) {
  PR_REQUIRE(h, "pr_hmr_set_streams: null handle");
  pr::DeviceGuard g(h->device);
  PR_TRY(pr::refuse_under_declared_capture("pr_hmr_set_streams"));
  return pr::set_chunks(h, std::min(n_streams, h->max_batch));
}

}

namespace pr {
namespace {
int encode_batch(pr_hmr_t* h, const float* x_dev, int B, hipStream_t s, int stop_block, void* tap) {
  int sizes[4096];
  bool concurrent = false;
  const int nsub = hmr_split_batch(B, h->chunk_cap, h->n_chunks, h->profile != 0, sizes, 4096, &concurrent);
  const size_t frame = (size_t)3 * kImg * kImg;
  const size_t tap_frame = stop_block >= 0 ? block_frame_elems(stop_block) * (h->precision == 1 ? 2 : 4) : 0;
  auto tap_at = [&](int b0) { return tap ? (void*)((char*)tap + (size_t)b0 * tap_frame) : nullptr; };
  if (!concurrent) {
    for (int i = 0, b0 = 0; i < nsub; b0 += sizes[i], ++i) {
      ChunkRun r{0, x_dev + b0 * frame, sizes[i], h->xf + (size_t)b0 * 2048, s, tap_at(b0)};
      PR_TRY(encode_chunks(h, &r, 1, stop_block));
    }
  } else {
    const int nch = nsub;
    ChunkRun runs[pr_hmr::kMaxChunks];
    PR_HIP(hipEventRecord(h->ev_fork, s));
    for (int c = 0, b0 = 0; c < nch; b0 += sizes[c], ++c) {
      runs[c] = ChunkRun{c, x_dev + b0 * frame, sizes[c], h->xf + (size_t)b0 * 2048, h->streams[c], tap_at(b0)};
      PR_HIP(hipStreamWaitEvent(h->streams[c], h->ev_fork, 0));
    }
    PR_TRY(encode_chunks(h, runs, nch, stop_block));
    for (int c = 0; c < nch; ++c) {
      PR_HIP(hipEventRecord(h->ev_join[c], h->streams[c]));
      PR_HIP(hipStreamWaitEvent(s, h->ev_join[c], 0));
    }
  }
  return PR_OK;
}

int regress_steps(pr_hmr_t* h, const float* xf, int B, int last, hipStream_t s) {
  PR_TRY(launch_state_init(h->init157, h->state, B, s));
  if (last < 1) return PR_OK;
  PR_TRY(fc_launch(h, h->fc1x, xf, nullptr, h->h_static, B, true, s));
  for (int it = 0; it < 3; ++it) {
    if (last < 2 + 3 * it) return PR_OK;
    PR_TRY(fc_launch(h, h->fc1s, h->state, h->h_static, h->h1, B, false, s));
    if (last < 3 + 3 * it) return PR_OK;
    PR_TRY(fc_launch(h, h->fc2, h->h1, nullptr, h->h2, B, true, s));
    if (last < 4 + 3 * it) return PR_OK;
    PR_TRY(fc_launch(h, h->dec, h->h2, h->state, h->state, B, true, s));
  }
  return PR_OK;
}
}
}

extern "C" {

int pr_hmr_forward(pr_hmr_t* h, const float* x_dev, int B, float* rotmat_dev, float* betas_dev,
                   float* cam_dev, float* xf_dev, float* pose6d_dev, void* stream) {
  using namespace pr;
  PR_REQUIRE(B >= 0, "pr_hmr_forward: negative batch");
  if (B == 0) return PR_OK;
  PR_REQUIRE(h && x_dev, "pr_hmr_forward: null argument");
  if (B > h->max_batch) {
    set_error("pr_hmr_forward: batch %d exceeds max_batch %d", B, h->max_batch);
    return PR_ERR_CAPACITY;
  }
  if (B == 0) return PR_OK;
  hipStream_t s = (hipStream_t)stream;
  PR_TRY(encode_batch(h, x_dev, B, s, -1, nullptr));
  if (xf_dev) PR_HIP(hipMemcpyAsync(xf_dev, h->xf, (size_t)B * 2048 * sizeof(float), hipMemcpyDeviceToDevice, s));
  if (!rotmat_dev && !betas_dev && !cam_dev && !pose6d_dev) return PR_OK;
  PR_TRY(regress_steps(h, h->xf, B, 10, s));
  PR_TRY(launch_regressor_finalize(h->state, rotmat_dev, betas_dev, cam_dev, pose6d_dev, B, s));
  return PR_OK;
}

int pr_hmr_encode_until(pr_hmr_t* h, const float* x_dev, int B, int block, void* act_dev, void* stream) {
  using namespace pr;
  PR_REQUIRE(B >= 1, "pr_hmr_encode_until: batch %d out of range", B);
  PR_REQUIRE(block >= 0 && block < HmrPlan::kBlocks, "pr_hmr_encode_until: block %d out of range 0..%d", block,
             HmrPlan::kBlocks - 1);
  PR_REQUIRE(h && x_dev && act_dev, "pr_hmr_encode_until: null argument");
  PR_REQUIRE(B <= h->max_batch, "pr_hmr_encode_until: batch %d out of range 1..%d", B, h->max_batch);
  hipStream_t s = (hipStream_t)stream;
  PR_TRY(refuse_if_capturing(s, "pr_hmr_encode_until"));
  return encode_batch(h, x_dev, B, s, block, act_dev);
}

int pr_hmr_regress_until(pr_hmr_t* h, const float* xf_dev, int B, int step, float* out_dev, void* stream) {
  using namespace pr;
  PR_REQUIRE(B >= 1, "pr_hmr_regress_until: batch %d out of range", B);
  PR_REQUIRE(step >= 0 && step <= 10, "pr_hmr_regress_until: step %d out of range 0..10", step);
  PR_REQUIRE(h && xf_dev && out_dev, "pr_hmr_regress_until: null argument");
  PR_REQUIRE(B <= h->max_batch, "pr_hmr_regress_until: batch %d out of range 1..%d", B, h->max_batch);
  hipStream_t s = (hipStream_t)stream;
  PR_TRY(refuse_if_capturing(s, "pr_hmr_regress_until"));
  PR_TRY(regress_steps(h, xf_dev, B, step, s));
  const int phase = step < 2 ? step : 2 + (step - 2) % 3;
  const float* src = phase == 0 || phase == 4 ? h->state : phase == 1 ? h->h_static : phase == 2 ? h->h1 : h->h2;
  const size_t cols = phase == 0 || phase == 4 ? kStateStride : 1024;
  PR_HIP(hipMemcpyAsync(out_dev, src, (size_t)B * cols * sizeof(float), hipMemcpyDeviceToDevice, s));
  return PR_OK;
}

int pr_hmr_conv_form(pr_hmr_t* h) { return h ? h->conv_form : PR_ERR_INVALID; }

int pr_hmr_plan_counts(pr_hmr_t* h, int B, int* conv_launches, int* winograd_layers) {
  using namespace pr;
  PR_REQUIRE(h && B > 0 && B <= h->max_batch, "pr_hmr_plan_counts: need a handle and a batch within its capacity");
  hmr_plan_counts(*h, B, h->chunk_cap, h->n_chunks, h->profile != 0, conv_launches, winograd_layers);
  return PR_OK;
}

int pr_hmr_profile_enable(pr_hmr_t* h, int on) {
  PR_REQUIRE(h, "pr_hmr_profile_enable: null handle");
  h->profile = on != 0;
  return PR_OK;
}

int pr_hmr_profile_read(pr_hmr_t* h, float* ms, int* launches, double* flops_per_frame, double* mfma_flops_per_frame,
                        int n_layers) {
  using namespace pr;
  PR_REQUIRE(h && n_layers == kNumConv, "pr_hmr_profile_read: need %d layers", kNumConv);
  for (size_t i = 0; i < h->pending.size(); ++i) {
    float t = 0.f;
    PR_HIP(hipEventSynchronize(h->pending[i].second));
    PR_HIP(hipEventElapsedTime(&t, h->pending[i].first, h->pending[i].second));
    h->prof_ms[h->pending_layer[i]] += t;
    h->prof_n[h->pending_layer[i]] += 1;
    (void)hipEventDestroy(h->pending[i].first);
    (void)hipEventDestroy(h->pending[i].second);
  }
  h->pending.clear();
  h->pending_layer.clear();
  for (int i = 0; i < kNumConv; ++i) {
    if (ms) ms[i] = h->prof_ms[i];
    if (launches) launches[i] = h->prof_n[i];
    if (flops_per_frame) flops_per_frame[i] = 0.0;
    if (mfma_flops_per_frame) mfma_flops_per_frame[i] = 0.0;
    h->prof_ms[i] = 0.f;
    h->prof_n[i] = 0;
  }
  for (const ConvSpec& c : h->convs) {
    if (flops_per_frame) flops_per_frame[c.layer] = 2.0 * c.macs_per_frame();
    if (mfma_flops_per_frame) {
      mfma_flops_per_frame[c.layer] = 2.0 * c.mfma_macs_per_frame(h->precision == 1 ? 64 : kConvBK);
      if (c.out_hw && h->precision == 0 && h->stem_s2d && h->fuse_stem)
        mfma_flops_per_frame[c.layer] = 2.0 * (double)c.Ho() * c.Wo() * c.Cout * 156.0;
    }
  }
  return PR_OK;
}

}
```

poserisk_release_amd/csrc/host_plan.cc:

```cpp
#include "host_plan.h"

#include <algorithm>
#include <cmath>
#include <cstdlib>
#include <cstring>
#include <memory>
#include <vector>

namespace pr {

int conv_kpad_bf16(int K) { return ceil_div(K, 64) * 64; }

unsigned short f32_to_bf16_host(float f) {
  unsigned u;
  memcpy(&u, &f, 4);
  if ((u & 0x7fffffffu) > 0x7f800000u) return (unsigned short)((u >> 16) | 0x40);
  return (unsigned short)((u + 0x7fffu + ((u >> 16) & 1u)) >> 16);
}

void conv_pack_weights_bf16(const float* w, const double* scale, int Cout, int Cin_real, int cin_pad, int KH,
                            int KW, unsigned short* out) {
  const int Kpad = conv_kpad_bf16(KH * KW * cin_pad);
  for (int o = 0; o < Cout; ++o) {
    unsigned short* row = out + (size_t)o * Kpad;
    for (int k = 0; k < Kpad; ++k) row[k] = 0;
    const double s = scale ? scale[o] : 1.0;
    for (int ci = 0; ci < Cin_real; ++ci)
      for (int kh = 0; kh < KH; ++kh)
        for (int kw = 0; kw < KW; ++kw)
          row[conv_k_index_bf16(kh * KW + kw, ci, KH * KW, cin_pad)] =
              f32_to_bf16_host((float)((double)w[(((size_t)o * Cin_real + ci) * KH + kh) * KW + kw] * s));
  }
}

void conv_pack_weights(const float* w, const double* scale, int Cout, int Cin_real, int cin_pad,
                       int KH, int KW, float* out) {
  const int K = KH * KW * cin_pad;
  const int Kpad = ceil_div(K, kConvBK) * kConvBK;
  for (int o = 0; o < Cout; ++o) {
    float* row = out + (size_t)o * Kpad;
    for (int k = 0; k < Kpad; ++k) row[k] = 0.f;
    const double s = scale ? scale[o] : 1.0;
    for (int ci = 0; ci < Cin_real; ++ci)
      for (int kh = 0; kh < KH; ++kh)
        for (int kw = 0; kw < KW; ++kw) {
          const double v = (double)w[(((size_t)o * Cin_real + ci) * KH + kh) * KW + kw] * s;
          row[(kh * KW + kw) * cin_pad + ci] = (float)v;
        }
  }
}

void conv_winograd_pack_weights(const float* w, const double* scale, int Cout, int Cin, int form, float* out) {
  static const double G2[4][3] = {{1, 0, 0}, {0.5, 0.5, 0.5}, {0.5, -0.5, 0.5}, {0, 0, 1}};
  static const double G4[6][3] = {{1.0 / 4, 0, 0},          {-1.0 / 6, -1.0 / 6, -1.0 / 6}, {-1.0 / 6, 1.0 / 6, -1.0 / 6},
                                  {1.0 / 24, 1.0 / 12, 1.0 / 6}, {1.0 / 24, -1.0 / 12, 1.0 / 6},  {0, 0, 1}};
  double G5[6][3];
  {
    const double a = kWa, b = kWb, a2 = a * a, b2 = b * b, Na = 2 * a2 * (a2 - b2), Nb = 2 * b2 * (b2 - a2);
    const double rows[6][3] = {{1 / (a2 * b2), 0, 0}, {1 / Na, a / Na, a2 / Na}, {1 / Na, -a / Na, a2 / Na},
                               {1 / Nb, b / Nb, b2 / Nb}, {1 / Nb, -b / Nb, b2 / Nb}, {0, 0, 1}};
    for (int i = 0; i < 6; ++i)
      for (int j = 0; j < 3; ++j) G5[i][j] = rows[i][j];
  }
  const int m = conv_winograd_tile(form);
  const int n = m + 2;
  const double(*G)[3] = form == 5 ? G5 : m == 4 ? G4 : G2;
  for (int o = 0; o < Cout; ++o)
    for (int ci = 0; ci < Cin; ++ci) {
      const float* g = w + ((size_t)o * Cin + ci) * 9;
      const double sc = scale ? scale[o] : 1.0;
      double t[6][3];
      for (int i = 0; i < n; ++i)
        for (int j = 0; j < 3; ++j)
          t[i][j] = G[i][0] * ((double)g[j] * sc) + G[i][1] * ((double)g[3 + j] * sc) + G[i][2] * ((double)g[6 + j] * sc);
      for (int i = 0; i < n; ++i)
        for (int j = 0; j < n; ++j) {
          const double u = t[i][0] * G[j][0] + t[i][1] * G[j][1] + t[i][2] * G[j][2];
          out[((size_t)(n * i + j) * Cout + o) * Cin + ci] = (float)u;
        }
    }
}

void bottleneck_pack_rows_bf16(const unsigned short* src, int rows, int K, unsigned short* dst) {
  for (int o = 0; o < rows; ++o) {
    const int T = o >> 5, i = o & 31;
    const int sigma = 16 * ((i >> 2) & 1) + 4 * (i >> 3) + (i & 3);
    memcpy(dst + (size_t)o * K, src + (size_t)(32 * T + sigma) * K, (size_t)K * 2);
  }
}

void bottleneck256_pack_w2_frags_bf16(const unsigned short* rows, unsigned short* dst) {
  constexpr int kP = 256;
  for (int st = 0; st < 72; ++st)
    for (int cp = 0; cp < 4; ++cp)
      for (int c = 0; c < 2; ++c)
        for (int ks = 0; ks < 2; ++ks)
          for (int l = 0; l < 64; ++l) {
            const int i = l & 31, h = l >> 5;
            const unsigned short* src = rows + (size_t)(32 * (2 * cp + c) + i) * (9 * kP) + 32 * st + 16 * ks + 8 * h;
            std::copy(src, src + 8, dst + (((((size_t)st * 4 + cp) * 2 + c) * 2 + ks) * 64 + l) * 8);
          }
}

void bottleneck256_pack_w3_frags_bf16(const unsigned short* rows, unsigned short* dst) {
  constexpr int kP = 256;
  for (int cq = 0; cq < 16; ++cq)
    for (int c = 0; c < 2; ++c)
      for (int ks = 0; ks < 16; ++ks)
        for (int l = 0; l < 64; ++l) {
          const int i = l & 31, h = l >> 5;
          const unsigned short* src = rows + (size_t)(32 * (2 * cq + c) + i) * kP + 16 * ks + 8 * h;
          std::copy(src, src + 8, dst + ((((size_t)cq * 2 + c) * 16 + ks) * 64 + l) * 8);
        }
}

bool expand_res_bf16_fits(int K, int N) { return (K == 128 && N == 512) || (K == 256 && N == 1024); }
bool expand_dual_bf16_fits(int K1, int K2, int N) { return K1 == 128 && K2 == 256 && N == 512; }
bool bottleneck256_bf16_fits(int H, int W) { return H >= 1 && W >= 1 && H * W <= 224; }

namespace {

struct BlobReader {
  const float* p;
  size_t left;
  const float* take(size_t n) {
    if (n > left) return nullptr;
    const float* r = p;
    p += n;
    left -= n;
    return r;
  }
};

size_t hmr_weight_floats_impl() {
  size_t n = 64 * 3 * 49 + 4 * 64;
  int inpl = 64;
  const int planes[4] = {64, 128, 256, 512}, blocks[4] = {3, 4, 6, 3};
  for (int L = 0; L < 4; ++L)
    for (int b = 0; b < blocks[L]; ++b) {
      const int pl = planes[L];
      n += (size_t)pl * inpl + 4 * pl;
      n += (size_t)pl * pl * 9 + 4 * pl;
      n += (size_t)pl * 4 * pl + 4 * pl * 4;
      if (b == 0) n += (size_t)pl * 4 * inpl + 4 * pl * 4;
      inpl = pl * 4;
    }
  n += (size_t)1024 * 2205 + 1024 + (size_t)1024 * 1024 + 1024;
  n += (size_t)144 * 1024 + 144 + 10 * 1024 + 10 + 3 * 1024 + 3 + 144 + 10 + 3;
  return n;
}

struct Ctx {
  HmrPlan* h;
  PlanSink* sink;
};

int upload(Ctx& cx, const std::vector<float>& host, float** out) {
  return cx.sink->upload(host.data(), host.size() * sizeof(float), out);
}

int dev_alloc(Ctx& cx, size_t floats, float** out) { return cx.sink->zeros(std::max<size_t>(floats, 4) * sizeof(float), out); }

struct FoldedConv {
  const float* w = nullptr;
  std::vector<double> scale, bias;
};

int read_conv_bn(BlobReader& br, int Cout, int Cin_real, int k, FoldedConv* out) {
  out->w = br.take((size_t)Cout * Cin_real * k * k);
  const float* g = br.take(Cout);
  const float* be = br.take(Cout);
  const float* mu = br.take(Cout);
  const float* var = br.take(Cout);
  PR_REQUIRE(out->w && g && be && mu && var, "hmr: weight blob too short");
  out->scale.resize(Cout);
  out->bias.resize(Cout);
  for (int o = 0; o < Cout; ++o) {
    const double s = (double)g[o] / std::sqrt((double)var[o] + kBnEps);
    out->scale[o] = s;
    out->bias[o] = (double)be[o] - (double)mu[o] * s;
  }
  return PR_OK;
}

int packed_k(const HmrPlan* h, int K) { return h->precision == 1 ? conv_kpad_bf16(K) : ceil_div(K, kConvBK) * kConvBK; }

int upload_packed(Ctx& cx, const ConvSpec& spec, const FoldedConv& f1, const FoldedConv* f2, float** out) {
  HmrPlan* const h = cx.h;
  const int K1 = packed_k(h, spec.k * spec.k * spec.Cin), K2 = f2 ? packed_k(h, spec.Cin2) : 0;
  if (h->precision == 1) {
    std::vector<unsigned short> a((size_t)spec.Cout * K1), b((size_t)spec.Cout * K2), packed((size_t)spec.Cout * (K1 + K2));
    conv_pack_weights_bf16(f1.w, f1.scale.data(), spec.Cout, spec.Cin_real, spec.Cin, spec.k, spec.k, a.data());
    if (f2) conv_pack_weights_bf16(f2->w, f2->scale.data(), spec.Cout, spec.Cin2, spec.Cin2, 1, 1, b.data());
    for (int o = 0; o < spec.Cout; ++o) {
      memcpy(&packed[(size_t)o * (K1 + K2)], &a[(size_t)o * K1], (size_t)K1 * 2);
      if (K2) memcpy(&packed[(size_t)o * (K1 + K2) + K1], &b[(size_t)o * K2], (size_t)K2 * 2);
    }
    std::vector<float> as_f((packed.size() + 1) / 2);
    memcpy(as_f.data(), packed.data(), packed.size() * 2);
    return upload(cx, as_f, out);
  }
  std::vector<float> a((size_t)spec.Cout * K1), b((size_t)spec.Cout * K2), packed((size_t)spec.Cout * (K1 + K2));
  conv_pack_weights(f1.w, f1.scale.data(), spec.Cout, spec.Cin_real, spec.Cin, spec.k, spec.k, a.data());
  if (f2) conv_pack_weights(f2->w, f2->scale.data(), spec.Cout, spec.Cin2, spec.Cin2, 1, 1, b.data());
  for (int o = 0; o < spec.Cout; ++o) {
    memcpy(&packed[(size_t)o * (K1 + K2)], &a[(size_t)o * K1], (size_t)K1 * 4);
    if (K2) memcpy(&packed[(size_t)o * (K1 + K2) + K1], &b[(size_t)o * K2], (size_t)K2 * 4);
  }
  return upload(cx, packed, out);
}

int add_conv(Ctx& cx, BlobReader& br, ConvSpec spec, bool second = false) {
  HmrPlan* const h = cx.h;
  FoldedConv f1, f2;
  std::vector<float> s2d_w;
  if (spec.out_hw) {
    PR_TRY(read_conv_bn(br, spec.Cout, 3, 7, &f1));
    s2d_w.assign((size_t)spec.Cout * 12 * 16, 0.f);
    for (int o = 0; o < spec.Cout; ++o)
      for (int c = 0; c < 3; ++c)
        for (int kh = 0; kh < 7; ++kh)
          for (int kw = 0; kw < 7; ++kw) {
            const int th = (kh + 1) >> 1, di = (kh + 1) & 1, tw = (kw + 1) >> 1, dj = (kw + 1) & 1;
            s2d_w[(((size_t)o * 12 + (2 * di + dj) * 3 + c) * 4 + th) * 4 + tw] = f1.w[(((size_t)o * 3 + c) * 7 + kh) * 7 + kw];
          }
    f1.w = s2d_w.data();
  } else
  PR_TRY(read_conv_bn(br, spec.Cout, spec.Cin_real, spec.k, &f1));
  if (second) PR_TRY(read_conv_bn(br, spec.Cout, spec.Cin2, 1, &f2));
  std::vector<float> bias(spec.Cout);
  for (int o = 0; o < spec.Cout; ++o) bias[o] = (float)(f1.bias[o] + (second ? f2.bias[o] : 0.0));
  PR_TRY(upload_packed(cx, spec, f1, second ? &f2 : nullptr, &spec.w));
  PR_TRY(upload(cx, bias, &spec.bias));
  const float* w = f1.w;
  const std::vector<double>& scale = f1.scale;
  const int use_wino = h->stage_form[spec.stage];
  if (use_wino && h->precision == 0 && spec.k == 3 && spec.stride == 1 && spec.pad == 1 && spec.Cin >= h->wino_min_c &&
      spec.Cin == spec.Cin_real) {
    const int m = conv_winograd_tile(use_wino), n2 = (m + 2) * (m + 2);
    std::vector<float> u((size_t)n2 * spec.Cout * spec.Cin);
    conv_winograd_pack_weights(w, scale.data(), spec.Cout, spec.Cin, use_wino, u.data());
    PR_TRY(upload(cx, u, &spec.u));
    spec.wino_m = m;
    spec.wino_form = use_wino;
    const size_t tiles = (size_t)((spec.H + m - 1) / m) * ((spec.W + m - 1) / m);
    h->wino_floats_per_frame = std::max(h->wino_floats_per_frame, n2 * tiles * ((size_t)spec.Cin + spec.Cout));
  }
  if (h->precision == 1 && h->expand_regs && spec.k == 1 && spec.stride == 1 && expand_res_bf16_fits(spec.Cin, spec.Cout) &&
      spec.res_buf >= 0 && spec.in2_buf < 0 && !second)
    spec.cfg = kConvCfgExpand;
  if (h->precision == 1 && h->expand_regs && spec.k == 1 && spec.stride == 1 && second && spec.in2_buf >= 0 && spec.res_buf < 0 &&
      expand_dual_bf16_fits(spec.Cin, spec.Cin2, spec.Cout))
    spec.cfg = kConvCfgExpand;
  if (h->precision == 0 && h->regw && spec.k == 1 && spec.stride == 1 && spec.in2_buf < 0 && !second &&
      (spec.Cin == 128 || spec.Cin == 256) && spec.Cin == spec.Cin_real && spec.Cout % 64 == 0 && spec.cfg < 0)
    spec.cfg = kConvCfgRegW;
  {
    const int bk = h->precision == 1 ? 64 : kConvBK;
    if (spec.k == 1 && spec.stride == 1 && spec.Cout > spec.Cin && spec.Cin + spec.Cin2 <= h->panel_max_k &&
        spec.Cin % bk == 0 && spec.Cin2 % bk == 0 && spec.cfg < 0)
      spec.cfg = kConvCfgPanel;
  }
  if (h->precision == 0 && h->splitk > 1 && !spec.wino_m && spec.cfg < 0 && spec.in2_buf < 0 && !spec.w3 && spec.Cout == 512 &&
      spec.Ho() == 7 && spec.Cin % kConvBK == 0 && (spec.k == 1 || spec.k == 3))
    spec.splitk = h->splitk;
  h->convs.push_back(spec);
  return PR_OK;
}

int make_fc(Ctx& cx, const float* w, const float* b, int N, int src_cols, int col0, int K_real,
            int Kpad, int Npad, FcSpec* out) {
  std::vector<float> packed((size_t)Npad * Kpad, 0.f), bias(Npad, 0.f);
  for (int n = 0; n < N; ++n) {
    for (int k = 0; k < K_real; ++k) packed[(size_t)n * Kpad + k] = w[(size_t)n * src_cols + col0 + k];
    if (b) bias[n] = b[n];
  }
  out->K = Kpad;
  out->N = Npad;
  PR_TRY(upload(cx, packed, &out->w));
  PR_TRY(upload(cx, bias, &out->bias));
  return PR_OK;
}

int build(Ctx& cx, const float* blob, size_t n_floats) {
  HmrPlan* const h = cx.h;
  BlobReader br{blob, n_floats};
  ConvSpec c1{3, h->precision == 1 ? 8 : 4, 64, 7, 2, 3, kImg, kImg, 1, 0, 1, -1};
  if (h->stem_s2d) {
    c1 = ConvSpec{12, h->precision == 1 ? 16 : 12, 64, 4, 1, 2, kImg / 2, kImg / 2, 1, 0, 1, -1};
    c1.out_hw = kImg / 2;
    c1.macs_fixed = (double)(kImg / 2) * (kImg / 2) * 64 * 3 * 49;
  }
  PR_TRY(add_conv(cx, br, c1));
  h->block_last[0] = 0;
  h->block_buf[0] = 2;
  int cur = 2, H = 56, inpl = 64, layer = 1, blk_no = 1;
  const int planes[4] = {64, 128, 256, 512}, blocks[4] = {3, 4, 6, 3};
  for (int L = 0; L < 4; ++L)
    for (int b = 0; b < blocks[L]; ++b) {
      const int pl = planes[L];
      const int stride = (b == 0 && L > 0) ? 2 : 1;
      int fr[4], nf = 0;
      for (int i = 1; i <= 5 && nf < 4; ++i)
        if (i != cur) fr[nf++] = i;
      const int t1 = fr[0], t2 = fr[1], ds = fr[2], outb = fr[3];
      const int Ho = H / stride;
      ConvSpec a{inpl, inpl, pl, 1, 1, 0, H, H, 1, cur, t1, -1};
      ConvSpec bb{pl, pl, pl, 3, stride, 1, H, H, 1, t1, t2, -1};
      ConvSpec cc{pl, pl, pl * 4, 1, 1, 0, Ho, Ho, 1, t2, outb, b == 0 ? ds : cur};
      a.stage = bb.stage = cc.stage = L;
      if (h->precision == 1 && ((L == 0 && h->fuse_bottleneck && (b > 0 || h->fuse_downsample)) ||
                                (L == 1 && b > 0 && h->fuse_bottleneck2))) {
        const bool first = b == 0;
        FoldedConv f1, f2, f3, fd;
        PR_TRY(read_conv_bn(br, pl, inpl, 1, &f1));
        PR_TRY(read_conv_bn(br, pl, pl, 3, &f2));
        PR_TRY(read_conv_bn(br, pl * 4, pl, 1, &f3));
        if (first) PR_TRY(read_conv_bn(br, pl * 4, inpl, 1, &fd));
        ConvSpec blk{inpl, inpl, pl * 4, 1, 1, 0, H, H, 1, cur, outb, -1};
        blk.stage = L;
        blk.bneck_planes = pl;
        blk.bneck_first = first;
        auto packed16 = [&](const FoldedConv& f, int Cout, int Cin, int k) {
          std::vector<unsigned short> a16((size_t)Cout * conv_kpad_bf16(k * k * Cin));
          conv_pack_weights_bf16(f.w, f.scale.data(), Cout, Cin, Cin, k, k, a16.data());
          return a16;
        };
        auto upload_rows = [&](const std::vector<unsigned short>& a16, int Cout, float** out) -> int {
          const int K = (int)(a16.size() / Cout);
          std::vector<unsigned short> p16(a16.size());
          bottleneck_pack_rows_bf16(a16.data(), Cout, K, p16.data());
          std::vector<float> as_f((p16.size() + 1) / 2);
          memcpy(as_f.data(), p16.data(), p16.size() * 2);
          return upload(cx, as_f, out);
        };
        auto bias_of = [&](const FoldedConv& f, const FoldedConv* g, float** out) -> int {
          std::vector<float> bv(f.bias.size());
          for (size_t o = 0; o < bv.size(); ++o) bv[o] = (float)(f.bias[o] + (g ? g->bias[o] : 0.0));
          return upload(cx, bv, out);
        };
        PR_TRY(upload_rows(packed16(f1, pl, inpl, 1), pl, &blk.w));
        PR_TRY(upload_rows(packed16(f2, pl, pl, 3), pl, &blk.w2b));
        if (first) {
          const std::vector<unsigned short> a3 = packed16(f3, pl * 4, pl, 1), ad = packed16(fd, pl * 4, inpl, 1);
          std::vector<unsigned short> both((size_t)pl * 4 * (pl + inpl));
          for (int o = 0; o < pl * 4; ++o) {
            memcpy(&both[(size_t)o * (pl + inpl)], &a3[(size_t)o * pl], (size_t)pl * 2);
            memcpy(&both[(size_t)o * (pl + inpl) + pl], &ad[(size_t)o * inpl], (size_t)inpl * 2);
          }
          PR_TRY(upload_rows(both, pl * 4, &blk.w3));
        } else {
          PR_TRY(upload_rows(packed16(f3, pl * 4, pl, 1), pl * 4, &blk.w3));
        }
        PR_TRY(bias_of(f1, nullptr, &blk.bias));
        PR_TRY(bias_of(f2, nullptr, &blk.bias2b));
        PR_TRY(bias_of(f3, first ? &fd : nullptr, &blk.bias3));
        layer += first ? 3 : 2;
        blk.layer = layer++;
        h->convs.push_back(blk);
        h->block_last[blk_no] = (int)h->convs.size() - 1;
        h->block_buf[blk_no++] = outb;
        cur = outb;
        H = Ho;
        inpl = pl * 4;
        continue;
      }
      const bool alt3 = h->precision == 1 && h->fuse_bottleneck3 && L == 2 && b > 0 && bottleneck256_bf16_fits(H, H);
      if (alt3) {
        BlobReader again = br;
        FoldedConv f1, f2, f3;
        PR_TRY(read_conv_bn(again, pl, inpl, 1, &f1));
        PR_TRY(read_conv_bn(again, pl, pl, 3, &f2));
        PR_TRY(read_conv_bn(again, pl * 4, pl, 1, &f3));
        HmrPlan::FusedBlock fb;
        fb.first = h->convs.size();
        fb.blk = ConvSpec{inpl, inpl, pl * 4, 1, 1, 0, H, H, 1, cur, outb, -1};
        fb.blk.stage = L;
        fb.blk.bneck_planes = pl;
        auto rows16 = [&](const FoldedConv& f, int Cout, int Cin, int k) {
          std::vector<unsigned short> a16((size_t)Cout * conv_kpad_bf16(k * k * Cin)), p16(a16.size());
          conv_pack_weights_bf16(f.w, f.scale.data(), Cout, Cin, Cin, k, k, a16.data());
          bottleneck_pack_rows_bf16(a16.data(), Cout, (int)(a16.size() / Cout), p16.data());
          return p16;
        };
        auto upload16 = [&](const std::vector<unsigned short>& p16, float** out) -> int {
          std::vector<float> as_f((p16.size() + 1) / 2);
          memcpy(as_f.data(), p16.data(), p16.size() * 2);
          return upload(cx, as_f, out);
        };
        auto bias_of = [&](const FoldedConv& f, float** out) -> int {
          std::vector<float> bv(f.bias.size());
          for (size_t o = 0; o < bv.size(); ++o) bv[o] = (float)f.bias[o];
          return upload(cx, bv, out);
        };
        PR_TRY(upload16(rows16(f1, pl, inpl, 1), &fb.blk.w));
        {
          const std::vector<unsigned short> r2 = rows16(f2, pl, pl, 3), r3 = rows16(f3, pl * 4, pl, 1);
          std::vector<unsigned short> g2(r2.size()), g3(r3.size());
          bottleneck256_pack_w2_frags_bf16(r2.data(), g2.data());
          bottleneck256_pack_w3_frags_bf16(r3.data(), g3.data());
          PR_TRY(upload16(g2, &fb.blk.w2b));
          PR_TRY(upload16(g3, &fb.blk.w3));
        }
        PR_TRY(bias_of(f1, &fb.blk.bias));
        PR_TRY(bias_of(f2, &fb.blk.bias2b));
        PR_TRY(bias_of(f3, &fb.blk.bias3));
        h->fused3.push_back(fb);
      }
      a.layer = layer++;
      bb.layer = layer++;
      PR_TRY(add_conv(cx, br, a));
      PR_TRY(add_conv(cx, br, bb));
      if (b == 0 && h->fuse_downsample) {
        cc.res_buf = -1;
        cc.in2_buf = cur; cc.Cin2 = inpl; cc.H2 = H; cc.stride2 = stride;
        cc.layer2 = layer++;
        cc.layer = layer++;
        PR_TRY(add_conv(cx, br, cc, true));
      } else if (b == 0) {
        const size_t mark = h->convs.size();
        PR_TRY(add_conv(cx, br, cc));
        ConvSpec dd{inpl, inpl, pl * 4, 1, stride, 0, H, H, 0, cur, ds, -1};
        dd.stage = L;
        PR_TRY(add_conv(cx, br, dd));
        std::swap(h->convs[mark], h->convs[mark + 1]);
        h->convs[mark].layer = layer++;
        h->convs[mark + 1].layer = layer++;
      } else if (L == 0 && h->fuse_conv3) {
        FoldedConv f3;
        PR_TRY(read_conv_bn(br, cc.Cout, cc.Cin_real, 1, &f3));
        ConvSpec& f = h->convs.back();
        std::vector<float> bias3(cc.Cout);
        for (int o = 0; o < cc.Cout; ++o) bias3[o] = (float)f3.bias[o];
        PR_TRY(upload_packed(cx, cc, f3, nullptr, &f.w3));
        PR_TRY(upload(cx, bias3, &f.bias3));
        f.N3 = cc.Cout; f.res3_buf = cc.res_buf; f.out3_buf = cc.out_buf;
        f.layer2 = f.layer;
        f.layer = layer++;
      } else {
        cc.layer = layer++;
        PR_TRY(add_conv(cx, br, cc));
      }
      if (alt3) {
        PR_REQUIRE(h->convs.size() == h->fused3.back().first + 3, "hmr: a plain layer3 block is three launches of the plan");
        h->fused3.back().blk.layer = h->convs.back().layer;
      }
      h->block_last[blk_no] = (int)h->convs.size() - 1;
      h->block_buf[blk_no++] = outb;
      cur = outb;
      H = Ho;
      inpl = pl * 4;
    }
  h->final_buf = cur;
  PR_REQUIRE(blk_no == HmrPlan::kBlocks, "hmr: planned %d blocks", blk_no);
  PR_REQUIRE(layer == kNumConv && (int)h->convs.size() ==
                                      kNumConv - (h->fuse_downsample ? 4 : 0) -
                                          (h->precision == 1 && h->fuse_bottleneck ? (h->fuse_downsample ? 6 : 4) : h->fuse_conv3 ? 2 : 0) -
                                          (h->precision == 1 && h->fuse_bottleneck2 ? 6 : 0),
             "hmr: planned %d convolutions in %zu launches, expected %d", layer, h->convs.size(), kNumConv);

  const float* fc1w = br.take((size_t)1024 * 2205);
  const float* fc1b = br.take(1024);
  const float* fc2w = br.take((size_t)1024 * 1024);
  const float* fc2b = br.take(1024);
  const float* dpw = br.take((size_t)144 * 1024);
  const float* dpb = br.take(144);
  const float* dsw = br.take((size_t)10 * 1024);
  const float* dsb = br.take(10);
  const float* dcw = br.take((size_t)3 * 1024);
  const float* dcb = br.take(3);
  const float* ip = br.take(144);
  const float* is = br.take(10);
  const float* ic = br.take(3);
  PR_REQUIRE(fc1w && fc1b && fc2w && fc2b && dpw && dpb && dsw && dsb && dcw && dcb && ip && is && ic,
             "hmr: weight blob too short");
  PR_REQUIRE(br.left == 0, "hmr: weight blob has %zu trailing floats", br.left);
  PR_TRY(make_fc(cx, fc1w, fc1b, 1024, 2205, 0, 2048, 2048, 1024, &h->fc1x));
  PR_TRY(make_fc(cx, fc1w, nullptr, 1024, 2205, 2048, 157, kStateStride, 1024, &h->fc1s));
  PR_TRY(make_fc(cx, fc2w, fc2b, 1024, 1024, 0, 1024, 1024, 1024, &h->fc2));
  {
    std::vector<float> decw((size_t)157 * 1024), decb(157);
    std::copy(dpw, dpw + (size_t)144 * 1024, decw.begin());
    std::copy(dsw, dsw + (size_t)10 * 1024, decw.begin() + (size_t)144 * 1024);
    std::copy(dcw, dcw + (size_t)3 * 1024, decw.begin() + (size_t)154 * 1024);
    std::copy(dpb, dpb + 144, decb.begin());
    std::copy(dsb, dsb + 10, decb.begin() + 144);
    std::copy(dcb, dcb + 3, decb.begin() + 154);
    PR_TRY(make_fc(cx, decw.data(), decb.data(), 157, 1024, 0, 1024, 1024, kStateStride, &h->dec));
  }
  {
    std::vector<float> init(160, 0.f);
    std::copy(ip, ip + 144, init.begin());
    std::copy(is, is + 10, init.begin() + 144);
    std::copy(ic, ic + 3, init.begin() + 154);
    PR_TRY(upload(cx, init, &h->init157));
  }

  const size_t B = (size_t)h->max_batch;
  PR_TRY(dev_alloc(cx, B * 2048, &h->xf));
  PR_TRY(dev_alloc(cx, B * 1024, &h->h_static));
  PR_TRY(dev_alloc(cx, B * 1024, &h->h1));
  PR_TRY(dev_alloc(cx, B * 1024, &h->h2));
  PR_TRY(dev_alloc(cx, B * kStateStride, &h->state));
  return PR_OK;
}

}

size_t hmr_weight_floats() { return hmr_weight_floats_impl(); }

bool hmr_conv_form_valid(int conv_form) {
  auto form_ok = [](int f) { return f == 0 || f == 2 || f == 4 || f == 5; };
  return conv_form == PR_CONV_FORM_DEFAULT || form_ok(conv_form) ||
         (conv_form >= 100 && conv_form <= 555 && form_ok(conv_form / 100) && form_ok(conv_form / 10 % 10) && form_ok(conv_form % 10));
}

void hmr_plan_configure(HmrPlan* h, int precision, int conv_form, int max_batch) {
  auto form_ok = [](int f) { return f == 0 || f == 2 || f == 4 || f == 5; };
  h->max_batch = max_batch;
  h->precision = precision;
  if (conv_form == PR_CONV_FORM_DEFAULT) {
    conv_form = PR_CONV_FORM_BUILTIN_DEFAULT;
    if (const char* e = getenv("POSERISK_WINOGRAD")) {
      const int v = atoi(e);
      conv_form = (v == 2 || v == 4 || v == 5 || (v >= 100 && v <= 555)) ? v : 0;
    }
  }
  h->conv_form = conv_form;
  for (int st = 1; st < 4; ++st) {
    const int f = conv_form >= 100 ? (st == 1 ? conv_form / 100 : st == 2 ? conv_form / 10 % 10 : conv_form % 10) : conv_form;
    h->stage_form[st] = form_ok(f) ? f : 0;
  }
  if (const char* e = getenv("POSERISK_FC_TILES")) h->fc_tiles = atoi(e);
  if (const char* e = getenv("POSERISK_FC_SHAPE")) h->fc_shape = atoi(e);
  if (const char* e = getenv("POSERISK_WINOGRAD_MIN_C")) h->wino_min_c = atoi(e);
  if (const char* e = getenv("POSERISK_FUSE_DOWNSAMPLE")) h->fuse_downsample = atoi(e) != 0;
  if (const char* e = getenv("POSERISK_FUSE_CONV3")) h->fuse_conv3 = atoi(e) != 0;
  if (const char* e = getenv("POSERISK_STEM_S2D")) h->stem_s2d = atoi(e) != 0;
  if (const char* e = getenv("POSERISK_FUSE_BOTTLENECK")) h->fuse_bottleneck = atoi(e) != 0;
  if (const char* e = getenv("POSERISK_FUSE_BOTTLENECK2")) h->fuse_bottleneck2 = atoi(e) != 0;
  if (const char* e = getenv("POSERISK_FUSE_STEM")) h->fuse_stem = atoi(e) != 0;
  if (const char* e = getenv("POSERISK_EXPAND_REGS")) h->expand_regs = atoi(e) != 0;
  if (const char* e = getenv("POSERISK_FUSE_BOTTLENECK3")) h->fuse_bottleneck3 = atoi(e) != 0;
  if (const char* e = getenv("POSERISK_B128_LEAD")) h->b128_lead = atoi(e);
  if (const char* e = getenv("POSERISK_BALANCED")) h->balanced = atoi(e) != 0;
  if (precision == 1) h->panel_max_k = 0;
  if (const char* e = getenv("POSERISK_PANEL_MAX_K")) h->panel_max_k = atoi(e);
  if (const char* e = getenv("POSERISK_REGW")) h->regw = atoi(e) != 0;
  if (const char* e = getenv("POSERISK_SPLITK")) h->splitk = std::max(1, std::min(atoi(e), 8));
}

int hmr_plan_build(HmrPlan* plan, const float* blob, size_t n_floats, PlanSink& sink) {
  PR_REQUIRE(plan && blob, "hmr plan: null argument");
  PR_REQUIRE(n_floats == hmr_weight_floats(), "pr_hmr_create: blob has %zu floats, expected %zu", n_floats, hmr_weight_floats());
  PR_REQUIRE(plan->max_batch > 0 && plan->max_batch <= 4096, "pr_hmr_create: max_batch %d out of range", plan->max_batch);
  Ctx cx{plan, &sink};
  return build(cx, blob, n_floats);
}

HmrChunkSizes hmr_chunk_sizes(const HmrPlan& plan, int chunk_cap) {
  HmrChunkSizes z{};
  const size_t cb = (size_t)chunk_cap;
  const size_t fmap = (size_t)112 * 112 * 64;
  z.act0_floats = cb * kImg * kImg * 4;
  z.act_floats = plan.precision == 1 ? (cb * fmap + 1) / 2 : cb * fmap;
  z.wino_floats = cb * plan.wino_floats_per_frame;
  for (const ConvSpec& cs : plan.convs)
    if (cs.splitk > 1) {
      const size_t tiles = (size_t)ceil_div((int)(cb * cs.Ho() * cs.Wo()), 64) * (cs.Cout / 64);
      z.slab_floats = std::max(z.slab_floats, tiles * cs.splitk * 4096);
      z.tickets = std::max(z.tickets, tiles);
    }
  return z;
}

int hmr_split_batch(int B, int chunk_cap, int n_chunks, bool serial, int* sizes, int max_sizes, bool* concurrent) {
  int nch = serial ? 1 : std::min(n_chunks, B);
  if (nch > 1 && ceil_div(B, nch) > chunk_cap) nch = 1;
  int n = 0;
  if (nch <= 1) {
    for (int b0 = 0; b0 < B && n < max_sizes; b0 += chunk_cap) sizes[n++] = std::min(chunk_cap, B - b0);
  } else {
    for (int c = 0; c < nch && n < max_sizes; ++c) sizes[n++] = (int)((long)(c + 1) * B / nch) - (int)((long)c * B / nch);
  }
  if (concurrent) *concurrent = nch > 1;
  return n;
}

void hmr_plan_counts(const HmrPlan& plan, int B, int chunk_cap, int n_chunks, bool serial, int* conv_launches, int* winograd_layers) {
  std::vector<int> sizes((size_t)std::max(n_chunks, ceil_div(std::max(B, 1), std::max(chunk_cap, 1))) + 1);
  const int n = hmr_split_batch(B, chunk_cap, n_chunks, serial, sizes.data(), (int)sizes.size(), nullptr);
  int launches = 0, wino = 0;
  for (int i = 0; i < n; ++i) {
    const bool fused3 = hmr_fused3_pays(sizes[i], plan.cus);
    size_t skip_until = 0;
    for (size_t ci = 0; ci < plan.convs.size(); ++ci) {
      if (ci < skip_until) continue;
      bool alt = false;
      for (const HmrPlan::FusedBlock& fb : plan.fused3) alt = alt || fb.first == ci;
      ++launches;
      if (alt && fused3) {
        skip_until = ci + 3;
        continue;
      }
      if (plan.convs[ci].u) ++wino;
    }
  }
  if (conv_launches) *conv_launches = launches;
  if (winograd_layers) *winograd_layers = wino;
}

}
```

poserisk_release_amd/csrc/host_plan.h:

```cpp
#pragma once
#include <algorithm>
#include <cstdlib>
#include <vector>

#include "host_common.h"

namespace pr {

constexpr int kConvBK = 32;
constexpr int kStateStride = 192;
constexpr int kImg = 224;
constexpr double kBnEps = 1e-5;
constexpr int kNumConv = 53;
constexpr int kHmrMaxChunks = 8;

constexpr int kConvCfgPanel = 100;
constexpr int kConvCfgExpand = 300;
constexpr int kConvCfgBalanced = 301;
constexpr int kConvCfgRegW = 400;

void conv_pack_weights(const float* w_oihw, const double* scale, int Cout, int Cin_real, int cin_pad, int KH, int KW,
                       float* out_packed);
void conv_pack_weights_bf16(const float* w_oihw, const double* scale, int Cout, int Cin_real, int cin_pad, int KH, int KW,
                            unsigned short* out_packed);
int conv_kpad_bf16(int K);
inline int conv_k_index_bf16(int tap, int ci, int taps, int cin_pad) {
  if (taps > 1 && cin_pad % 64 == 0) return (ci >> 6) * taps * 64 + tap * 64 + (ci & 63);
  return tap * cin_pad + ci;
}
unsigned short f32_to_bf16_host(float f);

constexpr float kWa = 11.f / 16.f, kWb = 3.f / 2.f;
inline int conv_winograd_tile(int form) { return form == 2 ? 2 : 4; }
void conv_winograd_pack_weights(const float* w_oihw, const double* scale, int Cout, int Cin, int form, float* out_u);

void bottleneck_pack_rows_bf16(const unsigned short* src, int rows, int K, unsigned short* dst);
void bottleneck256_pack_w2_frags_bf16(const unsigned short* rows, unsigned short* dst);
void bottleneck256_pack_w3_frags_bf16(const unsigned short* rows, unsigned short* dst);

bool expand_res_bf16_fits(int K, int N);
bool expand_dual_bf16_fits(int K1, int K2, int N);
bool bottleneck256_bf16_fits(int H, int W);

struct ConvSpec {
  int Cin_real, Cin, Cout, k, stride, pad, H, W;
  int relu;
  int in_buf, out_buf, res_buf;
  float* w = nullptr;
  float* bias = nullptr;
  float* u = nullptr;
  int wino_m = 0;
  int wino_form = 0;
  int cfg = -1;
  int layer = 0;
  int stage = 0;
  int in2_buf = -1, Cin2 = 0, H2 = 0, stride2 = 1, layer2 = -1;
  float* w3 = nullptr;
  float* bias3 = nullptr;
  int N3 = 0, res3_buf = -1, out3_buf = -1;
  int out_hw = 0;
  double macs_fixed = 0;
  int splitk = 1;
  int bneck_planes = 0;
  bool bneck_first = false;
  float* w2b = nullptr;
  float* bias2b = nullptr;
  int Ho() const { return out_hw ? out_hw : (H + 2 * pad - k) / stride + 1; }
  int Wo() const { return out_hw ? out_hw : (W + 2 * pad - k) / stride + 1; }
  double macs_per_frame() const {
    if (bneck_planes)
      return (double)H * W * bneck_planes * bneck_planes * (bneck_first ? 18.0 : 17.0);
    return macs_fixed > 0 ? macs_fixed : (double)Ho() * Wo() * (Cout * (Cin_real * k * k + Cin2) + (double)N3 * Cout);
  }
  double mfma_macs_per_frame(int k_step) const {
    if (bneck_planes) return macs_per_frame();
    if (wino_m) {
      const double tiles = (double)((H + wino_m - 1) / wino_m) * ((W + wino_m - 1) / wino_m);
      return tiles * (wino_m + 2) * (wino_m + 2) * Cin * Cout;
    }
    const int kp = (k * k * Cin + k_step - 1) / k_step * k_step;
    return (double)Ho() * Wo() * (Cout * (double)(kp + Cin2) + (double)N3 * Cout);
  }
};

struct FcSpec {
  int K = 0, N = 0;
  float* w = nullptr;
  float* bias = nullptr;
};

struct PlanSink {
  virtual int upload(const void* host, size_t bytes, float** out) = 0;
  virtual int zeros(size_t bytes, float** out) = 0;
  virtual ~PlanSink() = default;
};

struct HmrPlan {
  int max_batch = 0;
  int precision = 0;
  int conv_form = PR_CONV_FORM_BUILTIN_DEFAULT;
  int stage_form[4] = {0, 5, 5, 5};
  int wino_min_c = 128;
  bool fuse_downsample = true;
  bool fuse_conv3 = true;
  bool expand_regs = true;
  bool balanced = true;
  int cus = 256;
  bool fuse_stem = true;
  bool fuse_bottleneck = true;
  bool fuse_bottleneck2 = true;
  bool fuse_bottleneck3 = true;
  int b128_lead = 2;
  bool stem_s2d = true;
  bool regw = true;
  int panel_max_k = 128;
  int splitk = 1;
  int fc_tiles = 0;
  int fc_shape = 0;
  std::vector<ConvSpec> convs;
  FcSpec fc1x, fc1s, fc2, dec;
  float* init157 = nullptr;
  size_t wino_floats_per_frame = 0;
  int final_buf = 0;
  struct FusedBlock {
    size_t first;
    ConvSpec blk;
  };
  std::vector<FusedBlock> fused3;
  static constexpr int kBlocks = 17;
  int block_last[kBlocks] = {};
  int block_buf[kBlocks] = {};
  float* xf = nullptr;
  float* h_static = nullptr;
  float* h1 = nullptr;
  float* h2 = nullptr;
  float* state = nullptr;
};

size_t hmr_weight_floats();
bool hmr_conv_form_valid(int conv_form);
void hmr_plan_configure(HmrPlan* plan, int precision, int conv_form, int max_batch);
int hmr_plan_build(HmrPlan* plan, const float* blob, size_t n_floats, PlanSink& sink);

inline bool hmr_fused3_pays(int b, int cus) {
  const int rounds = (b + cus - 1) / cus;
  return b > 0 && (long)b * 100 >= (long)rounds * cus * 85;
}
inline int hmr_chunk_cap(int max_batch, int n_chunks) { return std::min(ceil_div(max_batch, n_chunks), 512); }
struct HmrChunkSizes {
  size_t act0_floats, act_floats, wino_floats, slab_floats, tickets;
};
HmrChunkSizes hmr_chunk_sizes(const HmrPlan& plan, int chunk_cap);
void hmr_plan_counts(const HmrPlan& plan, int B, int chunk_cap, int n_chunks, bool serial, int* conv_launches, int* winograd_layers);
int hmr_split_batch(int B, int chunk_cap, int n_chunks, bool serial, int* sizes, int max_sizes, bool* concurrent);

}
```

poserisk_release_amd/ops.py:

```python
import numpy as np
import torch

from . import _lib


def _stream(dev):
    return torch.cuda.current_stream(dev).cuda_stream


def _need_cuda(t, name):
    if t.device.type != "cuda":
        raise _lib.PoseRiskHipError(f"{name}: tensor must be on the GPU (no CPU fallback)")


def rot6d_to_rotmat(pose6d):
    _need_cuda(pose6d, "rot6d_to_rotmat")
    p = pose6d.contiguous().float()
    N = p.shape[0]
    out = torch.empty((N, 24, 3, 3), dtype=torch.float32, device=p.device)
    _lib.check(_lib.load().pr_rot6d_to_rotmat(p.data_ptr(), N, out.data_ptr(), _stream(p.device)), "pr_rot6d_to_rotmat")
    return out


def pose_to_euler(rotmat):
    _need_cuda(rotmat, "pose_to_euler")
    r = rotmat.contiguous().float()
    N = r.shape[0]
    aa = torch.empty((N, 24, 3), dtype=torch.float32, device=r.device)
    eul = torch.empty((N, 24, 3), dtype=torch.float64, device=r.device)
    st = torch.empty((N,), dtype=torch.int32, device=r.device)
    _lib.check(_lib.load().pr_pose_to_euler(r.data_ptr(), N, aa.data_ptr(), eul.data_ptr(), st.data_ptr(),
                                            _stream(r.device)), "pr_pose_to_euler")
    return aa, eul, st


def axis_angle_to_euler(axis_angle):
    _need_cuda(axis_angle, "axis_angle_to_euler")
    a = axis_angle.contiguous().float()
    N = a.shape[0]
    eul = torch.empty((N, 24, 3), dtype=torch.float64, device=a.device)
    st = torch.empty((N,), dtype=torch.int32, device=a.device)
    _lib.check(_lib.load().pr_axis_angle_to_euler(a.data_ptr(), N, eul.data_ptr(), st.data_ptr(), _stream(a.device)),
               "pr_axis_angle_to_euler")
    return eul, st


def reba(euler_deg, info):
    _need_cuda(euler_deg, "reba")
    e = euler_deg.contiguous().double()
    N = e.shape[0]
    out = torch.empty((N, 10), dtype=torch.int32, device=e.device)
    s = _lib.reba_info_struct(info)
    _lib.check(_lib.load().pr_reba(e.data_ptr(), N, s, out.data_ptr(), _stream(e.device)), "pr_reba")
    return out


def rula(euler_deg, info):
    _need_cuda(euler_deg, "rula")
    e = euler_deg.contiguous().double()
    N = e.shape[0]
    out = torch.empty((N, 12), dtype=torch.int32, device=e.device)
    s = _lib.rula_info_struct(info)
    _lib.check(_lib.load().pr_rula(e.data_ptr(), N, s, out.data_ptr(), _stream(e.device)), "pr_rula")
    return out


def _out(out, shape, dt, dev):
    if out is None:
        return torch.empty(shape, dtype=dt, device=dev)
    if tuple(out.shape) != tuple(shape) or out.dtype != dt or not out.is_contiguous() or out.device != dev:
        raise ValueError(f"out must be a contiguous {dt} tensor of shape {tuple(shape)} on {dev}")
    return out


def conv2d_nhwc(x, w_oihw, bias=None, residual=None, stride=1, pad=0, relu=False, tile_cfg=-1, repeats=0,
                precision="fp32", out=None):
    _need_cuda(x, "conv2d_nhwc")
    bf = precision == "bf16"
    dt = torch.bfloat16 if bf else torch.float32
    x = x.contiguous().to(dt)
    B, H, W, Cin = x.shape
    w = np.ascontiguousarray(w_oihw, dtype=np.float32)
    Cout, Cin_real, KH, KW = w.shape
    Ho = (H + 2 * pad - KH) // stride + 1
    Wo = (W + 2 * pad - KW) // stride + 1
    y = _out(out, (B, Ho, Wo, Cout), dt, x.device)
    b = np.ascontiguousarray(bias, dtype=np.float32) if bias is not None else None
    res = residual.contiguous().to(dt) if residual is not None else None
    ms = np.zeros(1, np.float32)
    idx = x.device.index if x.device.index is not None else torch.cuda.current_device()
    _lib.check(_lib.load().pr_conv2d_nhwc(
        idx, x.data_ptr(), w.ctypes.data, b.ctypes.data if b is not None else None,
        res.data_ptr() if res is not None else None, y.data_ptr(), B, H, W, Cin, Cin_real, Cout, KH, KW,
        stride, pad, int(relu), tile_cfg, 1 if bf else 0, repeats, ms.ctypes.data, _stream(x.device)), "pr_conv2d_nhwc")
    return y, (float(ms[0]) if repeats > 0 else None)


def conv1x1_dual_nhwc(x1, w1, x2, w2, bias=None, stride2=1, relu=False, tile_cfg=-1, precision="fp32", out=None):
    _need_cuda(x1, "conv1x1_dual_nhwc")
    bf = precision == "bf16"
    dt = torch.bfloat16 if bf else torch.float32
    x1, x2 = x1.contiguous().to(dt), x2.contiguous().to(dt)
    B, Ho, Wo, C1 = x1.shape
    _, H2, W2, C2 = x2.shape
    w1 = np.ascontiguousarray(w1, dtype=np.float32).reshape(-1, C1)
    w2 = np.ascontiguousarray(w2, dtype=np.float32).reshape(-1, C2)
    Cout = w1.shape[0]
    y = _out(out, (B, Ho, Wo, Cout), dt, x1.device)
    b = np.ascontiguousarray(bias, dtype=np.float32) if bias is not None else None
    idx = x1.device.index if x1.device.index is not None else torch.cuda.current_device()
    _lib.check(_lib.load().pr_conv1x1_dual_nhwc(
        idx, x1.data_ptr(), w1.ctypes.data, x2.data_ptr(), w2.ctypes.data, b.ctypes.data if b is not None else None,
        y.data_ptr(), B, Ho, Wo, C1, H2, W2, C2, stride2, Cout, int(relu), tile_cfg, 1 if bf else 0,
        _stream(x1.device)), "pr_conv1x1_dual_nhwc")
    return y


def conv3x3_conv1x1_nhwc(x, w2, b2, w3, b3, residual=None, relu=True, precision="fp32", out=None):
    _need_cuda(x, "conv3x3_conv1x1_nhwc")
    bf = precision == "bf16"
    dt = torch.bfloat16 if bf else torch.float32
    x = x.contiguous().to(dt)
    B, H, W, Cin = x.shape
    w2 = np.ascontiguousarray(w2, dtype=np.float32)
    w3 = np.ascontiguousarray(w3, dtype=np.float32).reshape(-1, 64)
    b2 = np.ascontiguousarray(b2, dtype=np.float32)
    b3 = np.ascontiguousarray(b3, dtype=np.float32)
    N3 = w3.shape[0]
    res = residual.contiguous().to(dt) if residual is not None else None
    y = _out(out, (B, H, W, N3), dt, x.device)
    idx = x.device.index if x.device.index is not None else torch.cuda.current_device()
    _lib.check(_lib.load().pr_conv3x3_conv1x1_nhwc(
        idx, x.data_ptr(), w2.ctypes.data, b2.ctypes.data, w3.ctypes.data, b3.ctypes.data,
        res.data_ptr() if res is not None else None, y.data_ptr(), B, H, W, Cin, N3, int(relu), 1 if bf else 0,
        _stream(x.device)), "pr_conv3x3_conv1x1_nhwc")
    return y


def bottleneck_nhwc(x, w1, b1, w2, b2, w3, b3, wd=None, bd=None, repeats=0):
    _need_cuda(x, "bottleneck_nhwc")
    x = x.contiguous().to(torch.bfloat16)
    B, H, W, C = x.shape
    first = wd is not None
    if C != (64 if first else 256):
        raise ValueError(f"bottleneck_nhwc: {64 if first else 256} input channels expected, got {C}")
    f = lambda a, shape: np.ascontiguousarray(a, dtype=np.float32).reshape(shape)
    w1, w2, w3 = f(w1, (64, C)), f(w2, (64, 64, 3, 3)), f(w3, (256, 64))
    b1, b2, b3 = f(b1, (64,)), f(b2, (64,)), f(b3, (256,))
    if first:
        wd, bd = f(wd, (256, 64)), f(bd, (256,))
    y = torch.empty((B, H, W, 256), dtype=torch.bfloat16, device=x.device)
    ms = np.zeros(1, np.float32)
    idx = x.device.index if x.device.index is not None else torch.cuda.current_device()
    _lib.check(_lib.load().pr_bottleneck_nhwc(idx, x.data_ptr(), w1.ctypes.data, b1.ctypes.data, w2.ctypes.data,
                                              b2.ctypes.data, w3.ctypes.data, b3.ctypes.data,
                                              wd.ctypes.data if first else None, bd.ctypes.data if first else None,
                                              y.data_ptr(), B, H, W, repeats, ms.ctypes.data, _stream(x.device)),
               "pr_bottleneck_nhwc")
    return y, (float(ms[0]) if repeats > 0 else None)


def bottleneck128_nhwc(x, w1, b1, w2, b2, w3, b3, repeats=0):
    _need_cuda(x, "bottleneck128_nhwc")
    x = x.contiguous().to(torch.bfloat16)
    B, H, W, C = x.shape
    if C != 512:
        raise ValueError(f"bottleneck128_nhwc: 512 input channels expected, got {C}")
    f = lambda a, shape: np.ascontiguousarray(a, dtype=np.float32).reshape(shape)
    w1, w2, w3 = f(w1, (128, 512)), f(w2, (128, 128, 3, 3)), f(w3, (512, 128))
    b1, b2, b3 = f(b1, (128,)), f(b2, (128,)), f(b3, (512,))
    y = torch.empty((B, H, W, 512), dtype=torch.bfloat16, device=x.device)
    ms = np.zeros(1, np.float32)
    idx = x.device.index if x.device.index is not None else torch.cuda.current_device()
    _lib.check(_lib.load().pr_bottleneck128_nhwc(idx, x.data_ptr(), w1.ctypes.data, b1.ctypes.data, w2.ctypes.data,
                                                 b2.ctypes.data, w3.ctypes.data, b3.ctypes.data, y.data_ptr(), B, H, W,
                                                 repeats, ms.ctypes.data, _stream(x.device)), "pr_bottleneck128_nhwc")
    return y, (float(ms[0]) if repeats > 0 else None)


def bottleneck256_nhwc(x, w1, b1, w2, b2, w3, b3, repeats=0):
    _need_cuda(x, "bottleneck256_nhwc")
    x = x.contiguous().to(torch.bfloat16)
    B, H, W, C = x.shape
    if C != 1024:
        raise ValueError(f"bottleneck256_nhwc: 1024 input channels expected, got {C}")
    f = lambda a, shape: np.ascontiguousarray(a, dtype=np.float32).reshape(shape)
    w1, w2, w3 = f(w1, (256, 1024)), f(w2, (256, 256, 3, 3)), f(w3, (1024, 256))
    b1, b2, b3 = f(b1, (256,)), f(b2, (256,)), f(b3, (1024,))
    y = torch.empty((B, H, W, 1024), dtype=torch.bfloat16, device=x.device)
    ms = np.zeros(1, np.float32)
    idx = x.device.index if x.device.index is not None else torch.cuda.current_device()
    _lib.check(_lib.load().pr_bottleneck256_nhwc(idx, x.data_ptr(), w1.ctypes.data, b1.ctypes.data, w2.ctypes.data,
                                                 b2.ctypes.data, w3.ctypes.data, b3.ctypes.data, y.data_ptr(), B, H, W,
                                                 repeats, ms.ctypes.data, _stream(x.device)), "pr_bottleneck256_nhwc")
    return y, (float(ms[0]) if repeats > 0 else None)


def stem_pool_nhwc(x, w, bias, repeats=0):
    _need_cuda(x, "stem_pool_nhwc")
    x = x.contiguous().to(torch.bfloat16)
    B, H, W, C = x.shape
    if C != 16 or H != W or H % 2:
        raise ValueError("stem_pool_nhwc: x must be [B,H,H,16] with even H")
    w = np.ascontiguousarray(w, dtype=np.float32).reshape(64, 16, 4, 4)
    b = np.ascontiguousarray(bias, dtype=np.float32).reshape(64)
    y = torch.empty((B, H // 2, H // 2, 64), dtype=torch.bfloat16, device=x.device)
    ms = np.zeros(1, np.float32)
    idx = x.device.index if x.device.index is not None else torch.cuda.current_device()
    _lib.check(_lib.load().pr_stem_pool_nhwc(idx, x.data_ptr(), w.ctypes.data, b.ctypes.data, y.data_ptr(), B, H, repeats,
                                             ms.ctypes.data, _stream(x.device)), "pr_stem_pool_nhwc")
    return y, (float(ms[0]) if repeats > 0 else None)


def stem_pool_f32_nhwc(x, w, bias, repeats=0):
    _need_cuda(x, "stem_pool_f32_nhwc")
    x = x.contiguous().float()
    if tuple(x.shape[1:]) != (112, 112, 12):
        raise ValueError(f"stem_pool_f32_nhwc: x must be [B,112,112,12], got {tuple(x.shape)}")
    B = x.shape[0]
    w = np.ascontiguousarray(w, dtype=np.float32).reshape(64, 12, 4, 4)
    b = np.ascontiguousarray(bias, dtype=np.float32).reshape(64)
    y = torch.empty((B, 56, 56, 64), dtype=torch.float32, device=x.device)
    ms = np.zeros(1, np.float32)
    idx = x.device.index if x.device.index is not None else torch.cuda.current_device()
    _lib.check(_lib.load().pr_stem_pool_f32_nhwc(idx, x.data_ptr(), w.ctypes.data, b.ctypes.data, y.data_ptr(), B, repeats,
                                                 ms.ctypes.data, _stream(x.device)), "pr_stem_pool_f32_nhwc")
    return y, (float(ms[0]) if repeats > 0 else None)


def crop_frames(frames, bboxes, frame_idx=None, scale=1.2, bgr=False, return_status=False):
    _need_cuda(frames, "crop_frames")
    if frames.dtype != torch.uint8 or frames.dim() != 4 or frames.shape[3] != 3:
        raise ValueError("frames must be uint8 [F,H,W,3]")
    frames = frames.contiguous()
    bb = torch.as_tensor(bboxes, dtype=torch.float32).to(frames.device).contiguous()
    N = bb.shape[0]
    if frame_idx is None:
        if N > frames.shape[0]:
            raise ValueError(f"{N} boxes for {frames.shape[0]} frames without a frame index")
    else:
        if not (isinstance(frame_idx, torch.Tensor) and frame_idx.device.type == "cuda"):
            host = np.asarray(frame_idx).reshape(-1)
            if host.shape[0] != N:
                raise ValueError(f"{host.shape[0]} frame indices for {N} boxes")
            if N and (int(host.min()) < 0 or int(host.max()) >= frames.shape[0]):
                raise ValueError(f"frame index out of range: {int(host.min())}..{int(host.max())} with "
                                 f"{frames.shape[0]} frames")
    if bb.dim() != 2 or bb.shape[1] != 4:
        raise ValueError(f"bboxes must be [N,4] (cx,cy,w,h), got {tuple(bb.shape)}")
    idx = None
    if frame_idx is not None:
        idx = torch.as_tensor(frame_idx).to(frames.device)
        if idx.dim() != 1 or idx.numel() != N:
            raise ValueError(f"frame_idx must be a vector of {N} frame indices, got shape {tuple(idx.shape)}")
        if idx.dtype.is_floating_point or idx.dtype == torch.bool:
            raise ValueError(f"frame_idx must hold integers, got {idx.dtype}")
        idx = idx.to(torch.int32).contiguous()
    out = torch.empty((N, 3, 224, 224), dtype=torch.float32, device=frames.device)
    status = torch.empty((N,), dtype=torch.int32, device=frames.device) if return_status else None
    F, H, W, _ = frames.shape
    _lib.check(_lib.load().pr_crop_frames(frames.data_ptr(), F, H, W, int(bool(bgr)),
                                          idx.data_ptr() if idx is not None else None, bb.data_ptr(), N,
                                          float(scale), out.data_ptr(),
                                          status.data_ptr() if status is not None else None,
                                          _stream(frames.device)), "pr_crop_frames")
    return (out, status) if return_status else out
```

Before: 17280 frames/s.

## Add fused Winograd F(4x4,3x3) kernel for 64-channel layer1 convolutions

Measured after the change: 17580 frames/s, median of 6. 1.02x the previous value.

```diff
diff --git a/include/poserisk_hip.h b/include/poserisk_hip.h
--- a/include/poserisk_hip.h
+++ b/include/poserisk_hip.h
@@ -66,6 +66,10 @@
 int pr_conv3x3_conv1x1_nhwc(int device, const void* x_dev, const float* w2_host, const float* b2_host,
                             const float* w3_host, const float* b3_host, const void* res_dev, void* y_dev,
                             int B, int H, int W, int Cin, int N3, int relu3, int precision, void* stream);
+
+int pr_conv3x3_wino64_nhwc(int device, const void* x_dev, const float* w2_host, const float* b2_host,
+                           const float* w3_host, const float* b3_host, const void* res_dev, void* y_dev, int B, int H,
+                           int W, int Cin, int Cout, int N3, int relu2, int relu3, int form, void* stream);
 
 int pr_bottleneck_nhwc(int device, const void* x_dev, const float* w1_host, const float* b1_host, const float* w2_host,
                        const float* b2_host, const float* w3_host, const float* b3_host, const float* wd_host,
diff --git a/poserisk_release_amd/_lib.py b/poserisk_release_amd/_lib.py
--- a/poserisk_release_amd/_lib.py
+++ b/poserisk_release_amd/_lib.py
@@ -4,7 +4,7 @@
 HERE = os.path.dirname(os.path.abspath(__file__))
 LIB_PATH = os.environ.get("POSERISK_LIB_PATH") or os.path.join(HERE, "libposerisk_hip.so")
 
-ABI_VERSION = 13
+ABI_VERSION = 14
 
 
 class PoseRiskHipError(RuntimeError):
@@ -57,6 +57,7 @@
     "pr_conv2d_nhwc": (_I, [_I, _P, _P, _P, _P, _P] + [_I] * 14 + [_P, _P]),
     "pr_conv1x1_dual_nhwc": (_I, [_I, _P, _P, _P, _P, _P, _P] + [_I] * 12 + [_P]),
     "pr_conv3x3_conv1x1_nhwc": (_I, [_I, _P, _P, _P, _P, _P, _P, _P] + [_I] * 7 + [_P]),
+    "pr_conv3x3_wino64_nhwc": (_I, [_I, _P, _P, _P, _P, _P, _P, _P] + [_I] * 9 + [_P]),
     "pr_bottleneck_nhwc": (_I, [_I, _P, _P, _P, _P, _P, _P, _P, _P, _P, _P, _I, _I, _I, _I, _P, _P]),
     "pr_bottleneck128_nhwc": (_I, [_I, _P, _P, _P, _P, _P, _P, _P, _P, _I, _I, _I, _I, _P, _P]),
     "pr_bottleneck256_nhwc": (_I, [_I, _P, _P, _P, _P, _P, _P, _P, _P, _I, _I, _I, _I, _P, _P]),
diff --git a/poserisk_release_amd/csrc/capi.hip b/poserisk_release_amd/csrc/capi.hip
--- a/poserisk_release_amd/csrc/capi.hip
+++ b/poserisk_release_amd/csrc/capi.hip
@@ -29,7 +29,7 @@
 extern "C" {
 
 const char* pr_last_error(void) { return pr::g_last_error.c_str(); }
-int pr_abi_version(void) { return 13; }
+int pr_abi_version(void) { return 14; }
 
 int pr_declare_stream(void* stream, int declared) {
   pr::g_stream_declared = declared != 0;
@@ -290,6 +290,49 @@
   p.res3 = (const float*)res_dev; p.y3 = (float*)y_dev;
   p.N3 = N3; p.relu3 = relu3;
   const int st = conv_launch(p, 8, s);
+  const hipError_t e = hipStreamSynchronize(s);
+  if (st != PR_OK) return st;
+  PR_HIP(e);
+  return PR_OK;
+}
+
+int pr_conv3x3_wino64_nhwc(int device, const void* x_dev, const float* w2_host, const float* b2_host, const float* w3_host,
+                           const float* b3_host, const void* res_dev, void* y_dev, int B, int H, int W, int Cin, int Cout, int N3,
+                           int relu2, int relu3, int form, void* stream) {
+  using namespace pr;
+  PR_REQUIRE(x_dev && w2_host && b2_host && y_dev, "pr_conv3x3_wino64_nhwc: null argument");
+  PR_REQUIRE(Cin == 64 && Cout == 64, "pr_conv3x3_wino64_nhwc: Cin = Cout = 64 only (got %d -> %d)", Cin, Cout);
+  PR_REQUIRE(form == 4 || form == 5, "pr_conv3x3_wino64_nhwc: form %d is not 4 or 5", form);
+  PR_REQUIRE(B >= 0 && H > 0 && W > 0, "pr_conv3x3_wino64_nhwc: bad geometry");
+  PR_REQUIRE(!w3_host || (b3_host && N3 > 0 && N3 % 64 == 0), "pr_conv3x3_wino64_nhwc: conv3 needs a bias and N3 %% 64 == 0 (%d)", N3);
+  DeviceGuard g(device);
+  hipStream_t s = (hipStream_t)stream;
+  PR_TRY(refuse_if_capturing(s, "stand-alone test entry"));
+  struct Scratch {
+    float* p[4] = {nullptr, nullptr, nullptr, nullptr};
+    ~Scratch() {
+      for (float* q : p)
+        if (q) (void)hipFree(q);
+    }
+  } sc;
+  std::vector<float> u((size_t)36 * 64 * 64), up(u.size());
+  conv_winograd_pack_weights(w2_host, nullptr, 64, 64, form, u.data());
+  conv_wino64_pack_u(u.data(), up.data());
+  const size_t sizes[4] = {up.size(), 64, w3_host ? (size_t)N3 * 64 : 0, w3_host ? (size_t)N3 : 0};
+  const float* src[4] = {up.data(), b2_host, w3_host, b3_host};
+  for (int i = 0; i < 4; ++i) {
+    if (!sizes[i]) continue;
+    PR_HIP(hipMalloc(&sc.p[i], sizes[i] * sizeof(float)));
+    PR_HIP(hipMemcpy(sc.p[i], src[i], sizes[i] * sizeof(float), hipMemcpyHostToDevice));
+  }
+  ConvProblem p;
+  p.B = B; p.H = p.Ho = H; p.W = p.Wo = W; p.Cin = 64; p.Cout = 64; p.KH = p.KW = 3; p.stride = 1; p.pad = 1; p.relu = relu2;
+  p.precision = 0;
+  p.x = (const float*)x_dev; p.w = nullptr; p.bias = sc.p[1]; p.res = nullptr; p.y = w3_host ? nullptr : (float*)y_dev;
+  if (w3_host) {
+    p.w3 = sc.p[2]; p.bias3 = sc.p[3]; p.res3 = (const float*)res_dev; p.y3 = (float*)y_dev; p.N3 = N3; p.relu3 = relu3;
+  }
+  const int st = conv_wino64_launch(p, sc.p[0], form, s);
   const hipError_t e = hipStreamSynchronize(s);
   if (st != PR_OK) return st;
   PR_HIP(e);
diff --git a/poserisk_release_amd/csrc/conv_igemm.h b/poserisk_release_amd/csrc/conv_igemm.h
--- a/poserisk_release_amd/csrc/conv_igemm.h
+++ b/poserisk_release_amd/csrc/conv_igemm.h
@@ -64,6 +64,8 @@
 size_t conv_winograd_work_floats(const ConvProblem& p, int form);
 int conv_winograd_launch(const ConvProblem& p, const float* u, float* work, int form, hipStream_t stream);
 
+int conv_wino64_launch(const ConvProblem& p, const float* u, int form, hipStream_t stream);
+
 struct BottleneckProblem {
   const void* x = nullptr;
   void* y = nullptr;
diff --git a/poserisk_release_amd/csrc/conv_wino64.hip b/poserisk_release_amd/csrc/conv_wino64.hip
--- /dev/null
+++ b/poserisk_release_amd/csrc/conv_wino64.hip
@@ -0,0 +1,301 @@
+#include "conv_igemm.h"
+#include "wino_transforms.h"
+
+namespace pr {
+namespace {
+
+using f32x16 = __attribute__((ext_vector_type(16))) float;
+using f32x4 = __attribute__((ext_vector_type(4))) float;
+using u32x4 = __attribute__((ext_vector_type(4))) unsigned;
+
+[[maybe_unused]] constexpr unsigned kOOB = 0x80000000u;
+constexpr int kTiles = 16;
+constexpr int kSlice = 16;
+constexpr int kPlane = kTiles * kSlice;
+constexpr int kVBytes = 36 * kPlane * 4;
+[[maybe_unused]] constexpr int kRing = kVBytes;
+constexpr int kLdsPlain = kVBytes, kLdsFused = kVBytes + 2 * 8192;
+constexpr int kADepth = 2;
+static_assert(12 % kADepth == 0, "the ring position of a group must not depend on the slice");
+static_assert(2 * 16384 <= kVBytes, "the t2 image of eight tiles lies over the V image");
+
+struct WArgs {
+  const float* x;
+  const float* u;
+  const float* bias2;
+  const float* w3;
+  const float* bias3;
+  const float* res;
+  float* y;
+  unsigned x_bytes, y_bytes, w3_bytes;
+  int H, W, th, tcw, N3, relu, relu3;
+};
+
+__device__ __forceinline__ int v_pos(int tile, int g) { return g * 64 + ((4 * tile + 16 * g) & 63); }
+
+template <int PTS, bool FUSE3>
+__global__ __launch_bounds__(256, 2) void conv3x3_wino64_f32(const WArgs a) {
+#if defined(__HIP_DEVICE_COMPILE__)
+  extern __shared__ __attribute__((aligned(16))) char smem[];
+  const int unit = (int)xcd_contiguous_block(blockIdx.x, gridDim.x);
+  const int cc = unit % a.tcw, rowid = unit / a.tcw;
+  const int ty = rowid % a.th, img = rowid / a.th;
+  const int tx0 = cc * kTiles;
+  const int tid = threadIdx.x, lane = tid & 63;
+  const int wave = __builtin_amdgcn_readfirstlane(tid >> 6);
+  const auto xsrc = __builtin_amdgcn_make_buffer_rsrc(const_cast<float*>(a.x), 0, (int)a.x_bytes, 0x00020000);
+
+  const int pj = tid >> 4, pc = tid & 15;
+  const int h0 = 4 * ty - 1, w0 = 4 * (tx0 + pj) - 1;
+  const int pbase = (((img * a.H + h0) * a.W + w0) * 64 + pc) * 4;
+  bool hok[6], wok[6];
+#pragma unroll
+  for (int i = 0; i < 6; ++i) {
+    hok[i] = (unsigned)(h0 + i) < (unsigned)a.H;
+    wok[i] = (unsigned)(w0 + i) < (unsigned)a.W;
+  }
+  float* const vw = reinterpret_cast<float*>(smem) + v_pos(pj, pc >> 2) + (pc & 3);
+
+  const int j = lane & 15, g = lane >> 4;
+  const auto usrc = __builtin_amdgcn_make_buffer_rsrc(const_cast<float*>(a.u), 0, 36 * 64 * 64 * 4, 0x00020000);
+  const int ua = ((16 * wave + j) * kSlice + 4 * g) * 4;
+  const float* const vr = reinterpret_cast<const float*>(smem) + v_pos(j, g);
+  f32x4 y[4][4];
+#pragma unroll
+  for (int r = 0; r < 4; ++r)
+#pragma unroll
+    for (int c = 0; c < 4; ++c) y[r][c] = f32x4{0.f, 0.f, 0.f, 0.f};
+
+  auto load_patch = [&](float (&d)[6][6], int sl) {
+    int pb = pbase + sl * kSlice * 4;
+    asm volatile("" : "+v"(pb));
+#pragma unroll
+    for (int i = 0; i < 6; ++i)
+#pragma unroll
+      for (int jj = 0; jj < 6; ++jj)
+        d[i][jj] = __builtin_bit_cast(float, __builtin_amdgcn_raw_buffer_load_b32(
+                                                 xsrc, (hok[i] & wok[jj]) ? pb + (i * a.W + jj) * 256 : (int)kOOB, 0, 0));
+  };
+  f32x4 af[kADepth][3];
+  auto load_a = [&](int sl, int grp, int buf) {
+#pragma unroll
+    for (int t = 0; t < 3; ++t)
+      af[buf][t] = __builtin_bit_cast(f32x4, __builtin_amdgcn_raw_buffer_load_b128(usrc, ua, ((3 * grp + t) * 4 + sl) * (64 * kSlice * 4), 0));
+  };
+#pragma unroll
+  for (int gq = 0; gq + 1 < kADepth; ++gq) load_a(0, gq, gq);
+  for (int sl = 0; sl < 64 / kSlice; ++sl) {
+    float d[6][6];
+    load_patch(d, sl);
+    __builtin_amdgcn_sched_barrier(0);
+#pragma unroll
+    for (int jj = 0; jj < 6; ++jj) bt6<PTS>(d[0][jj], d[1][jj], d[2][jj], d[3][jj], d[4][jj], d[5][jj]);
+#pragma unroll
+    for (int i = 0; i < 6; ++i) bt6<PTS>(d[i][0], d[i][1], d[i][2], d[i][3], d[i][4], d[i][5]);
+    __syncthreads();
+#pragma unroll
+    for (int i = 0; i < 6; ++i)
+#pragma unroll
+      for (int jj = 0; jj < 6; ++jj) vw[(6 * i + jj) * kPlane] = d[i][jj];
+    __syncthreads();
+#pragma unroll
+    for (int i = 0; i < 6; ++i) {
+      __builtin_amdgcn_sched_barrier(0);
+      f32x4 m[6];
+#pragma unroll
+      for (int hh = 0; hh < 2; ++hh) {
+        const int grp = 2 * i + hh;
+        if (grp + kADepth - 1 < 12) load_a(sl, grp + kADepth - 1, (grp + kADepth - 1) % kADepth);
+        else if (sl + 1 < 64 / kSlice) load_a(sl + 1, grp + kADepth - 1 - 12, (grp + kADepth - 1) % kADepth);
+        f32x4 bf[3];
+#pragma unroll
+        for (int t = 0; t < 3; ++t) {
+          bf[t] = *reinterpret_cast<const f32x4*>(vr + (3 * grp + t) * kPlane);
+          m[3 * hh + t] = f32x4{0.f, 0.f, 0.f, 0.f};
+        }
+#pragma unroll
+        for (int e = 0; e < 4; ++e)
+#pragma unroll
+          for (int t = 0; t < 3; ++t)
+            m[3 * hh + t] = __builtin_amdgcn_mfma_f32_16x16x4f32(af[grp % kADepth][t][e], bf[t][e], m[3 * hh + t], 0, 0, 0);
+      }
+      f32x4 s[4];
+      at6<PTS>(m[0], m[1], m[2], m[3], m[4], m[5], s[0], s[1], s[2], s[3]);
+#pragma unroll
+      for (int r = 0; r < 4; ++r) {
+        constexpr float one = 1.f;
+        const float cf = at6_coef<PTS>(r, i);
+        if (cf == 0.f) continue;
+#pragma unroll
+        for (int c = 0; c < 4; ++c) y[r][c] = cf == one ? y[r][c] + s[c] : y[r][c] + cf * s[c];
+      }
+    }
+  }
+
+  const f32x4 b2 = *reinterpret_cast<const f32x4*>(a.bias2 + 16 * wave + 4 * g);
+  const auto ysrc = __builtin_amdgcn_make_buffer_rsrc(a.y, 0, (int)a.y_bytes, 0x00020000);
+  if constexpr (!FUSE3) {
+#pragma unroll
+    for (int r = 0; r < 4; ++r)
+#pragma unroll
+      for (int c = 0; c < 4; ++c) {
+        const int ho = 4 * ty + r, wo = 4 * (tx0 + j) + c;
+        f32x4 v = y[r][c] + b2;
+        if (a.relu) {
+#pragma unroll
+          for (int e = 0; e < 4; ++e) v[e] = fmaxf(v[e], 0.f);
+        }
+        const int off = (((img * a.H + ho) * a.W + wo) * 64 + 16 * wave + 4 * g) * 4;
+        __builtin_amdgcn_raw_buffer_store_b128(__builtin_bit_cast(u32x4, v), ysrc, ho < a.H && wo < a.W ? off : (int)kOOB, 0, 0);
+      }
+  } else {
+    const int wm = wave >> 1, wn = wave & 1;
+    const int q = (lane & 7) ^ ((4 * (wave & 1) + (lane >> 4)) & 7);
+    const auto w3src = __builtin_amdgcn_make_buffer_rsrc(const_cast<float*>(a.w3), 0, (int)a.w3_bytes, 0x00020000);
+    const auto rsrc = __builtin_amdgcn_make_buffer_rsrc(const_cast<float*>(a.res ? a.res : a.y), 0, (int)a.y_bytes, 0x00020000);
+    unsigned b3_off[2];
+#pragma unroll
+    for (int i = 0; i < 2; ++i) b3_off[i] = (unsigned)(((8 * (wave + 4 * i) + (lane >> 3)) * 64 + q * 4) * 4);
+    f32x4 wreg[2];
+    auto load3 = [&](int s) {
+      const int soff = ((s >> 1) * 64 * 64 + (s & 1) * kConvBK) * 4;
+#pragma unroll
+      for (int i = 0; i < 2; ++i)
+        wreg[i] = __builtin_bit_cast(f32x4, __builtin_amdgcn_raw_buffer_load_b128(w3src, (int)b3_off[i], soff, 0));
+    };
+    auto put3 = [&](int s) {
+      char* stage = smem + kRing + (s & 1) * 8192;
+#pragma unroll
+      for (int i = 0; i < 2; ++i) *reinterpret_cast<f32x4*>(stage + (wave + 4 * i) * 1024 + lane * 16) = wreg[i];
+    };
+    const int frow = lane & 31, fh = lane >> 5, fsw = (frow >> 1) & 7;
+    int foff[kConvBK / 8];
+#pragma unroll
+    for (int kk = 0; kk < kConvBK / 8; ++kk) foff[kk] = frow * 128 + (((2 * kk + fh) ^ fsw) << 4);
+    const int nsteps = (a.N3 >> 6) * 2;
+    const int col_l = lane & 31;
+    for (int hf = 0; hf < 2; ++hf) {
+      __syncthreads();
+      load3(0);
+      if ((j >> 3) == hf) {
+        char* t2 = smem + ((j & 7) >> 2) * 16384 + (wave >> 1) * 8192;
+#pragma unroll
+        for (int r = 0; r < 4; ++r)
+#pragma unroll
+          for (int c = 0; c < 4; ++c) {
+            const int row = 16 * (j & 3) + 4 * r + c;
+            f32x4 v = y[r][c] + b2;
+#pragma unroll
+            for (int e = 0; e < 4; ++e) v[e] = fmaxf(v[e], 0.f);
+            *reinterpret_cast<f32x4*>(t2 + row * 128 + (((4 * (wave & 1) + g) ^ ((row >> 1) & 7)) << 4)) = v;
+          }
+      }
+      int frag_off[2];
+      bool cok[2][2][4];
+      const int ho0 = 4 * ty + fh;
+#pragma unroll
+      for (int sub = 0; sub < 2; ++sub) {
+        const int wo0 = 4 * (tx0 + 8 * hf + 4 * sub + 2 * wm);
+        frag_off[sub] = (((img * a.H + ho0) * a.W + wo0) * a.N3 + wn * 32 + col_l) * 4;
+#pragma unroll
+        for (int t = 0; t < 2; ++t)
+#pragma unroll
+          for (int c = 0; c < 4; ++c) cok[sub][t][c] = wo0 + 4 * t + c < a.W;
+      }
+      const bool rok[2] = {ho0 < a.H, ho0 + 2 < a.H};
+      put3(0);
+      load3(1);
+      f32x16 acc[2];
+      float rfrag[2][16];
+      for (int s = 0; s < nsteps; ++s) {
+        __syncthreads();
+        if (s + 1 < nsteps) put3(s + 1);
+        if (s + 2 < nsteps) load3(s + 2);
+        const int n0 = (s >> 1) * 64;
+        if ((s & 1) == 0) {
+#pragma unroll
+          for (int sub = 0; sub < 2; ++sub) {
+#pragma unroll
+            for (int e = 0; e < 16; ++e) acc[sub][e] = 0.f;
+            if (a.res) {
+#pragma unroll
+              for (int e = 0; e < 16; ++e)
+                rfrag[sub][e] = __builtin_bit_cast(
+                    float, __builtin_amdgcn_raw_buffer_load_b32(
+                               rsrc, rok[(e >> 2) & 1] && cok[sub][e >> 3][e & 3] ? frag_off[sub] : (int)kOOB,
+                               (n0 + ((2 * ((e >> 2) & 1) * a.W + 4 * (e >> 3) + (e & 3)) * a.N3)) * 4, 0));
+            }
+          }
+        }
+        {
+          const char* Bb = smem + kRing + (s & 1) * 8192 + wn * 32 * 128;
+          const char* Ab = smem + (s & 1) * 8192 + wm * 32 * 128;
+          f32x4 af0[kConvBK / 8], af1[kConvBK / 8], bf[kConvBK / 8];
+#pragma unroll
+          for (int kk = 0; kk < kConvBK / 8; ++kk) {
+            af0[kk] = *reinterpret_cast<const f32x4*>(Ab + foff[kk]);
+            af1[kk] = *reinterpret_cast<const f32x4*>(Ab + 16384 + foff[kk]);
+            bf[kk] = *reinterpret_cast<const f32x4*>(Bb + foff[kk]);
+          }
+          __builtin_amdgcn_sched_barrier(0);
+#pragma unroll
+          for (int kk = 0; kk < kConvBK / 8; ++kk)
+#pragma unroll
+            for (int jx = 0; jx < 4; ++jx) {
+              acc[0] = __builtin_amdgcn_mfma_f32_32x32x2f32(af0[kk][jx], bf[kk][jx], acc[0], 0, 0, 0);
+              acc[1] = __builtin_amdgcn_mfma_f32_32x32x2f32(af1[kk][jx], bf[kk][jx], acc[1], 0, 0, 0);
+            }
+        }
+        if (s & 1) {
+          const float b3 = a.bias3[n0 + wn * 32 + col_l];
+#pragma unroll
+          for (int sub = 0; sub < 2; ++sub)
+#pragma unroll
+            for (int e = 0; e < 16; ++e) {
+              float v = acc[sub][e] + b3;
+              if (a.res) v += rfrag[sub][e];
+              if (a.relu3) v = fmaxf(v, 0.f);
+              __builtin_amdgcn_raw_buffer_store_b32(__builtin_bit_cast(unsigned, v), ysrc,
+                                                    rok[(e >> 2) & 1] && cok[sub][e >> 3][e & 3] ? frag_off[sub] : (int)kOOB,
+                                                    (n0 + ((2 * ((e >> 2) & 1) * a.W + 4 * (e >> 3) + (e & 3)) * a.N3)) * 4, 0);
+            }
+        }
+      }
+    }
+  }
+#endif
+}
+
+template <int PTS>
+int launch_pts(const WArgs& a, bool fuse3, int units, hipStream_t stream) {
+  if (fuse3) hipLaunchKernelGGL((conv3x3_wino64_f32<PTS, true>), dim3(units), dim3(256), kLdsFused, stream, a);
+  else hipLaunchKernelGGL((conv3x3_wino64_f32<PTS, false>), dim3(units), dim3(256), kLdsPlain, stream, a);
+  return check_launch("conv3x3_wino64_f32");
+}
+
+}
+
+int conv_wino64_launch(const ConvProblem& p, const float* u, int form, hipStream_t stream) {
+  PR_REQUIRE(form == 4 || form == 5, "conv_wino64: form %d (4 = F(4x4,3x3) on 0, +-1, +-2; 5 = on 0, +-11/16, +-3/2)", form);
+  PR_REQUIRE(p.precision == 0 && p.KH == 3 && p.KW == 3 && p.stride == 1 && p.pad == 1 && p.Ho == p.H && p.Wo == p.W && !p.res &&
+                 !p.x2 && p.groups == 1 && p.splitk == 1,
+             "conv_wino64: 3x3 / stride 1 / pad 1 fp32 convolutions without residual only");
+  PR_REQUIRE(p.Cin == 64 && p.Cout == 64, "conv_wino64: Cin = Cout = 64 only (got %d -> %d)", p.Cin, p.Cout);
+  PR_REQUIRE(p.x && u && p.bias && p.B >= 0 && p.H > 0 && p.W > 0, "conv_wino64: needs an input, U and a bias");
+  const bool fuse3 = p.w3 != nullptr;
+  if (fuse3) PR_REQUIRE(p.bias3 && p.y3 && p.N3 > 0 && p.N3 % 64 == 0, "conv_wino64: conv3 needs a bias and an output with N3 %% 64 == 0 (%d)", p.N3);
+  else PR_REQUIRE(p.y, "conv_wino64: null output");
+  const int nout = fuse3 ? p.N3 : 64;
+  const size_t xb = (size_t)p.B * p.H * p.W * 64 * 4, yb = (size_t)p.M() * nout * 4;
+  PR_REQUIRE(xb < (1ull << 31) && yb < (1ull << 31), "conv_wino64: tensor too large for one launch");
+  WArgs a;
+  a.x = p.x; a.u = u; a.bias2 = p.bias; a.w3 = p.w3; a.bias3 = p.bias3; a.res = fuse3 ? p.res3 : nullptr; a.y = fuse3 ? p.y3 : p.y;
+  a.x_bytes = (unsigned)xb; a.y_bytes = (unsigned)yb; a.w3_bytes = fuse3 ? (unsigned)((size_t)p.N3 * 64 * 4) : 0u;
+  a.H = p.H; a.W = p.W; a.th = (p.H + 3) / 4; a.tcw = ((p.W + 3) / 4 + kTiles - 1) / kTiles; a.N3 = p.N3; a.relu = p.relu; a.relu3 = p.relu3;
+  const long units = (long)p.B * a.th * a.tcw;
+  PR_REQUIRE(units < (1L << 31), "conv_wino64: %ld units are too many for one launch", units);
+  if (units == 0) return PR_OK;
+  return form == 5 ? launch_pts<1>(a, fuse3, (int)units, stream) : launch_pts<0>(a, fuse3, (int)units, stream);
+}
+
+}
diff --git a/poserisk_release_amd/csrc/conv_winograd.hip b/poserisk_release_amd/csrc/conv_winograd.hip
--- a/poserisk_release_amd/csrc/conv_winograd.hip
+++ b/poserisk_release_amd/csrc/conv_winograd.hip
@@ -1,6 +1,7 @@
 #include <algorithm>
 
 #include "conv_igemm.h"
+#include "wino_transforms.h"
 
 namespace pr {
 namespace {
@@ -103,29 +104,6 @@
 
 using f32x2 = __attribute__((ext_vector_type(2))) float;
 
-constexpr float kWa2 = kWa * kWa, kWb2 = kWb * kWb, kWab2 = kWa2 * kWb2, kWs2 = kWa2 + kWb2;
-
-template <int PTS, typename V>
-__device__ __forceinline__ void bt6(V& a0, V& a1, V& a2, V& a3, V& a4, V& a5) {
-  const V d0 = a0, d1 = a1, d2 = a2, d3 = a3, d4 = a4, d5 = a5;
-  if constexpr (PTS == 0) {
-    a0 = 4.f * d0 - 5.f * d2 + d4;
-    a1 = (d3 + d4) - 4.f * (d1 + d2);
-    a2 = 4.f * (d1 - d2) + (d4 - d3);
-    a3 = 2.f * (d3 - d1) + (d4 - d2);
-    a4 = 2.f * (d1 - d3) + (d4 - d2);
-    a5 = 4.f * d1 - 5.f * d3 + d5;
-  } else {
-    const V ea = d4 - kWb2 * d2, oa = kWa * (d3 - kWb2 * d1);
-    const V eb = d4 - kWa2 * d2, ob = kWb * (d3 - kWa2 * d1);
-    a0 = (kWab2 * d0 - kWs2 * d2) + d4;
-    a1 = ea + oa;
-    a2 = ea - oa;
-    a3 = eb + ob;
-    a4 = eb - ob;
-    a5 = (kWab2 * d1 - kWs2 * d3) + d5;
-  }
-}
 
 template <int PTS, typename V>
 __global__ __launch_bounds__(256) void wino43_input_transform(const WinoArgs a) {
@@ -161,21 +139,6 @@
   for (int i = 0; i < 6; ++i)
 #pragma unroll
     for (int j = 0; j < 6; ++j) *reinterpret_cast<V*>(out + (6 * i + j) * gs) = d[i][j];
-}
-
-template <int PTS, typename V>
-__device__ __forceinline__ void at6(const V m0, const V m1, const V m2, const V m3, const V m4, const V m5, V& o0, V& o1, V& o2, V& o3) {
-  const V s12 = m1 + m2, d12 = m1 - m2, s34 = m3 + m4, d34 = m3 - m4;
-  o0 = (m0 + s12) + s34;
-  if constexpr (PTS == 0) {
-    o1 = d12 + 2.f * d34;
-    o2 = s12 + 4.f * s34;
-    o3 = (d12 + 8.f * d34) + m5;
-  } else {
-    o1 = kWa * d12 + kWb * d34;
-    o2 = kWa2 * s12 + kWb2 * s34;
-    o3 = ((kWa2 * kWa) * d12 + (kWb2 * kWb) * d34) + m5;
-  }
 }
 
 template <int PTS, typename V>
diff --git a/poserisk_release_amd/csrc/hmr.hip b/poserisk_release_amd/csrc/hmr.hip
--- a/poserisk_release_amd/csrc/hmr.hip
+++ b/poserisk_release_amd/csrc/hmr.hip
@@ -206,6 +206,7 @@
           bp.lead_tiles = h->b128_lead;
           return bottleneck_bf16_launch(bp, r.s);
         }
+        if (c.u1) return conv_wino64_launch(p, c.u1, h->stage_form[0], r.s);
         return c.u ? conv_winograd_launch(p, c.u, h->wino_work[r.chunk], c.wino_form, r.s) : conv_launch(p, cfg, r.s);
       };
       if (h->profile) {
diff --git a/poserisk_release_amd/csrc/host_plan.cc b/poserisk_release_amd/csrc/host_plan.cc
--- a/poserisk_release_amd/csrc/host_plan.cc
+++ b/poserisk_release_amd/csrc/host_plan.cc
@@ -5,6 +5,7 @@
 #include <cstdlib>
 #include <cstring>
 #include <memory>
+#include <utility>
 #include <vector>
 
 namespace pr {
@@ -81,6 +82,12 @@
     }
 }
 
+void conv_wino64_pack_u(const float* u, float* out) {
+  for (int k = 0; k < 36; ++k)
+    for (int co = 0; co < 64; ++co)
+      for (int ci = 0; ci < 64; ++ci) out[(((size_t)k * 4 + (ci >> 4)) * 64 + co) * 16 + (ci & 15)] = u[((size_t)k * 64 + co) * 64 + ci];
+}
+
 void bottleneck_pack_rows_bf16(const unsigned short* src, int rows, int K, unsigned short* dst) {
   for (int o = 0; o < rows; ++o) {
     const int T = o >> 5, i = o & 31;
@@ -153,6 +160,8 @@
 struct Ctx {
   HmrPlan* h;
   PlanSink* sink;
+  std::vector<std::pair<size_t, std::vector<float>>> u1_pending;
+  int block = 0;
 };
 
 int upload(Ctx& cx, const std::vector<float>& host, float** out) {
@@ -235,7 +244,14 @@
   const float* w = f1.w;
   const std::vector<double>& scale = f1.scale;
   const int use_wino = h->stage_form[spec.stage];
-  if (use_wino && h->precision == 0 && spec.k == 3 && spec.stride == 1 && spec.pad == 1 && spec.Cin >= h->wino_min_c &&
+  if (spec.stage == 0 && use_wino && (h->wino_layer1 >= 2 || cx.block == 0) && h->precision == 0 && spec.k == 3 && spec.stride == 1 && spec.pad == 1 && spec.Cin == 64 &&
+      spec.Cout == 64 && spec.Cin == spec.Cin_real) {
+    std::vector<float> u((size_t)36 * 64 * 64), packed(u.size());
+    conv_winograd_pack_weights(w, scale.data(), 64, 64, use_wino, u.data());
+    conv_wino64_pack_u(u.data(), packed.data());
+    cx.u1_pending.emplace_back(h->convs.size(), std::move(packed));
+  }
+  if (spec.stage > 0 && use_wino && h->precision == 0 && spec.k == 3 && spec.stride == 1 && spec.pad == 1 && spec.Cin >= h->wino_min_c &&
       spec.Cin == spec.Cin_real) {
     const int m = conv_winograd_tile(use_wino), n2 = (m + 2) * (m + 2);
     std::vector<float> u((size_t)n2 * spec.Cout * spec.Cin);
@@ -300,6 +316,7 @@
     for (int b = 0; b < blocks[L]; ++b) {
       const int pl = planes[L];
       const int stride = (b == 0 && L > 0) ? 2 : 1;
+      cx.block = b;
       int fr[4], nf = 0;
       for (int i = 1; i <= 5 && nf < 4; ++i)
         if (i != cur) fr[nf++] = i;
@@ -452,6 +469,7 @@
       inpl = pl * 4;
     }
   h->final_buf = cur;
+  for (const auto& pu : cx.u1_pending) PR_TRY(upload(cx, pu.second, &h->convs[pu.first].u1));
   PR_REQUIRE(blk_no == HmrPlan::kBlocks, "hmr: planned %d blocks", blk_no);
   PR_REQUIRE(layer == kNumConv && (int)h->convs.size() ==
                                       kNumConv - (h->fuse_downsample ? 4 : 0) -
@@ -548,6 +566,8 @@
   if (const char* e = getenv("POSERISK_PANEL_MAX_K")) h->panel_max_k = atoi(e);
   if (const char* e = getenv("POSERISK_REGW")) h->regw = atoi(e) != 0;
   if (const char* e = getenv("POSERISK_SPLITK")) h->splitk = std::max(1, std::min(atoi(e), 8));
+  if (const char* e = getenv("POSERISK_WINO_LAYER1")) h->wino_layer1 = std::max(0, std::min(atoi(e), 2));
+  h->stage_form[0] = precision == 0 && h->wino_layer1 && (h->stage_form[1] == 4 || h->stage_form[1] == 5) ? h->stage_form[1] : 0;
 }
 
 int hmr_plan_build(HmrPlan* plan, const float* blob, size_t n_floats, PlanSink& sink) {
diff --git a/poserisk_release_amd/csrc/host_plan.h b/poserisk_release_amd/csrc/host_plan.h
--- a/poserisk_release_amd/csrc/host_plan.h
+++ b/poserisk_release_amd/csrc/host_plan.h
@@ -33,6 +33,8 @@
 constexpr float kWa = 11.f / 16.f, kWb = 3.f / 2.f;
 inline int conv_winograd_tile(int form) { return form == 2 ? 2 : 4; }
 void conv_winograd_pack_weights(const float* w_oihw, const double* scale, int Cout, int Cin, int form, float* out_u);
+constexpr int kWino64Tiles = 16;
+void conv_wino64_pack_u(const float* u, float* out);
 
 void bottleneck_pack_rows_bf16(const unsigned short* src, int rows, int K, unsigned short* dst);
 void bottleneck256_pack_w2_frags_bf16(const unsigned short* rows, unsigned short* dst);
@@ -51,6 +53,7 @@
   float* u = nullptr;
   int wino_m = 0;
   int wino_form = 0;
+  float* u1 = nullptr;
   int cfg = -1;
   int layer = 0;
   int stage = 0;
@@ -74,6 +77,10 @@
   }
   double mfma_macs_per_frame(int k_step) const {
     if (bneck_planes) return macs_per_frame();
+    if (u1) {
+      const int cols = ((W + 3) / 4 + kWino64Tiles - 1) / kWino64Tiles * kWino64Tiles;
+      return (double)((H + 3) / 4) * cols * 36 * Cin * Cout + (double)Ho() * Wo() * N3 * Cout;
+    }
     if (wino_m) {
       const double tiles = (double)((H + wino_m - 1) / wino_m) * ((W + wino_m - 1) / wino_m);
       return tiles * (wino_m + 2) * (wino_m + 2) * Cin * Cout;
@@ -101,6 +108,7 @@
   int conv_form = PR_CONV_FORM_BUILTIN_DEFAULT;
   int stage_form[4] = {0, 5, 5, 5};
   int wino_min_c = 128;
+  int wino_layer1 = 1;
   bool fuse_downsample = true;
   bool fuse_conv3 = true;
   bool expand_regs = true;
diff --git a/poserisk_release_amd/csrc/wino_transforms.h b/poserisk_release_amd/csrc/wino_transforms.h
--- /dev/null
+++ b/poserisk_release_amd/csrc/wino_transforms.h
@@ -0,0 +1,54 @@
+#pragma once
+#include "host_plan.h"
+
+namespace pr {
+
+constexpr float kWa2 = kWa * kWa, kWb2 = kWb * kWb, kWab2 = kWa2 * kWb2, kWs2 = kWa2 + kWb2;
+
+template <int PTS, typename V>
+__device__ __forceinline__ void bt6(V& a0, V& a1, V& a2, V& a3, V& a4, V& a5) {
+  const V d0 = a0, d1 = a1, d2 = a2, d3 = a3, d4 = a4, d5 = a5;
+  if constexpr (PTS == 0) {
+    a0 = 4.f * d0 - 5.f * d2 + d4;
+    a1 = (d3 + d4) - 4.f * (d1 + d2);
+    a2 = 4.f * (d1 - d2) + (d4 - d3);
+    a3 = 2.f * (d3 - d1) + (d4 - d2);
+    a4 = 2.f * (d1 - d3) + (d4 - d2);
+    a5 = 4.f * d1 - 5.f * d3 + d5;
+  } else {
+    const V ea = d4 - kWb2 * d2, oa = kWa * (d3 - kWb2 * d1);
+    const V eb = d4 - kWa2 * d2, ob = kWb * (d3 - kWa2 * d1);
+    a0 = (kWab2 * d0 - kWs2 * d2) + d4;
+    a1 = ea + oa;
+    a2 = ea - oa;
+    a3 = eb + ob;
+    a4 = eb - ob;
+    a5 = (kWab2 * d1 - kWs2 * d3) + d5;
+  }
+}
+
+template <int PTS, typename V>
+__device__ __forceinline__ void at6(const V m0, const V m1, const V m2, const V m3, const V m4, const V m5, V& o0, V& o1, V& o2, V& o3) {
+  const V s12 = m1 + m2, d12 = m1 - m2, s34 = m3 + m4, d34 = m3 - m4;
+  o0 = (m0 + s12) + s34;
+  if constexpr (PTS == 0) {
+    o1 = d12 + 2.f * d34;
+    o2 = s12 + 4.f * s34;
+    o3 = (d12 + 8.f * d34) + m5;
+  } else {
+    o1 = kWa * d12 + kWb * d34;
+    o2 = kWa2 * s12 + kWb2 * s34;
+    o3 = ((kWa2 * kWa) * d12 + (kWb2 * kWb) * d34) + m5;
+  }
+}
+
+template <int PTS>
+__host__ __device__ constexpr float at6_coef(int r, int i) {
+  const float a = PTS == 0 ? 1.f : kWa, b = PTS == 0 ? 2.f : kWb;
+  if (i == 0) return r == 0 ? 1.f : 0.f;
+  if (i == 5) return r == 3 ? 1.f : 0.f;
+  const float p = i == 1 ? a : i == 2 ? -a : i == 3 ? b : -b;
+  return r == 0 ? 1.f : r == 1 ? p : r == 2 ? p * p : p * p * p;
+}
+
+}
diff --git a/poserisk_release_amd/ops.py b/poserisk_release_amd/ops.py
--- a/poserisk_release_amd/ops.py
+++ b/poserisk_release_amd/ops.py
@@ -134,6 +134,28 @@
         idx, x.data_ptr(), w2.ctypes.data, b2.ctypes.data, w3.ctypes.data, b3.ctypes.data,
         res.data_ptr() if res is not None else None, y.data_ptr(), B, H, W, Cin, N3, int(relu), 1 if bf else 0,
         _stream(x.device)), "pr_conv3x3_conv1x1_nhwc")
+    return y
+
+
+def conv3x3_wino64_nhwc(x, w2, b2, w3=None, b3=None, residual=None, relu=True, form=5, out=None):
+    _need_cuda(x, "conv3x3_wino64_nhwc")
+    x = x.contiguous().float()
+    B, H, W, Cin = x.shape
+    w2 = np.ascontiguousarray(w2, dtype=np.float32)
+    b2 = np.ascontiguousarray(b2, dtype=np.float32)
+    Cout = w2.shape[0]
+    fused = w3 is not None
+    if fused:
+        w3 = np.ascontiguousarray(w3, dtype=np.float32).reshape(-1, 64)
+        b3 = np.ascontiguousarray(b3, dtype=np.float32)
+    N3 = w3.shape[0] if fused else 0
+    res = residual.contiguous().float() if residual is not None else None
+    y = _out(out, (B, H, W, N3 if fused else Cout), torch.float32, x.device)
+    idx = x.device.index if x.device.index is not None else torch.cuda.current_device()
+    _lib.check(_lib.load().pr_conv3x3_wino64_nhwc(
+        idx, x.data_ptr(), w2.ctypes.data, b2.ctypes.data, w3.ctypes.data if fused else None,
+        b3.ctypes.data if fused else None, res.data_ptr() if res is not None else None, y.data_ptr(), B, H, W, Cin, Cout,
+        N3, int(relu), int(relu), form, _stream(x.device)), "pr_conv3x3_wino64_nhwc")
     return y
 
 
```
